# vacp2p/zerokit

Measured on AMD Instinct MI355X. Metric: RLN Groth16 proofs/sec (BN254, h=20), higher is better.
Workload: dtype u32 limbs (256-bit Montgomery integers, BN254 Fr/Fq; 8x32 and 9x29 forms)

## Files before the change

### zerokit_amd/csrc/prover.hip

```cpp
#include "prover.h"

#include <fcntl.h>
#include <stdlib.h>
#include <string.h>
#include <sys/stat.h>
#include <time.h>
#include <unistd.h>

#include <algorithm>
#include <atomic>
#include <chrono>
#include <deque>
#include <mutex>
#include <thread>

#include "prover_kernels.h"
#include "prover_plan.h"
#include "fq29.h"
#include "glv.h"
#include "pairing.h"
#include "poseidon.h"
#include "witness_ops.h"
#include "witness_lanes.h"
#include "witness_sched.h"
#include "fin29.h"

namespace rlnamd {

const char* const kProverStageNames[PROVER_STAGES] = {"witness", "matvec", "ntt",      "recode",
                                                      "msm_g1",  "msm_g2", "finalize", "values"};

struct Slot {
  DevBuf<uint32_t> err, coords, values;
  DevBuf<uint8_t> comp;
  DevBuf<Fr> V, abc;
  DevBuf<uint4> V29;
  DevBuf<int16_t> digits, digits2;
  DevBuf<G1XYZZ> part1, grp1, sums1, prod, tbl;
  DevBuf<G2XYZZ> part2, grp2, sums2;
  DevBuf<G1Affine> affA, affB1;
  DevBuf<G2Affine> affB2;
  DevBuf<uint32_t> pp_out;
  uint32_t* h_pp = nullptr;
  int mode = 0;
  DevBuf<uint32_t> inputs, rs, pp_in;
  uint8_t* h_in = nullptr;
  uint32_t* h_cone = nullptr;
  uint32_t* h_hints = nullptr;
  bool hinted = false;
  hipEvent_t evU = nullptr;
  hipEvent_t evE = nullptr;
  uint64_t ticket = 0;
  uint8_t* h_comp = nullptr;
  uint32_t* h_values = nullptr;
  uint32_t* h_err = nullptr;
  hipEvent_t evA = nullptr, evB = nullptr, evB2 = nullptr, evR = nullptr, evC = nullptr, evW = nullptr, evV = nullptr;
  hipEvent_t evX = nullptr;
  hipEvent_t evP = nullptr;
  DevBuf<uint4> pp_pow;
  hipEvent_t t[15] = {};
  bool used = false;
  bool marked = false;
  bool wiped = false;
  hipEvent_t evZ = nullptr;
  hipEvent_t free_event() const { return wiped ? evZ : evC; }
  size_t n = 0;
  uint32_t dB = 0, PB = 0, nch1 = 0, nch2 = 0;
};

static std::atomic<int> g_provers_on_device[64];

struct DeviceNeighbours {
  int fd = -1;
  void open_for(int dev) {
    char bus[64] = {0};
    if (hipDeviceGetPCIBusId(bus, sizeof bus, dev) != hipSuccess) {
      (void)hipGetLastError();
      return;
    }
    for (char* c = bus; *c; c++)
      if (*c == ':' || *c == '.') *c = '_';
    const std::string path = std::string("/dev/shm/rlnamd_") + bus + ".lock";
    fd = ::open(path.c_str(), O_RDWR | O_CREAT | O_CLOEXEC, 0666);
    if (fd < 0) return;
    (void)fchmod(fd, 0666);
    struct flock fl {};
    fl.l_type = F_RDLCK;
    fl.l_whence = SEEK_SET;
    fl.l_start = 0;
    fl.l_len = 1;
    if (fcntl(fd, F_SETLK, &fl) != 0) {
      ::close(fd);
      fd = -1;
    }
  }
  bool other_process() const {
    if (fd < 0) return false;
    struct flock fl {};
    fl.l_type = F_WRLCK;
    fl.l_whence = SEEK_SET;
    fl.l_start = 0;
    fl.l_len = 1;
    return fcntl(fd, F_GETLK, &fl) == 0 && fl.l_type != F_UNLCK;
  }
};
static std::mutex g_neigh_mu;
static DeviceNeighbours g_neigh[64];
static int g_neigh_users[64];

struct DeviceCount {
  int dev = -1;
  mutable std::chrono::steady_clock::time_point probed{};
  mutable bool other = false;
  DeviceCount() = default;
  DeviceCount(const DeviceCount&) = delete;
  DeviceCount& operator=(const DeviceCount&) = delete;
  void take() {
    int d = 0;
    if (hipGetDevice(&d) == hipSuccess && d >= 0 && d < 64) {
      dev = d;
      g_provers_on_device[d]++;
      std::lock_guard<std::mutex> lk(g_neigh_mu);
      if (g_neigh_users[d]++ == 0) g_neigh[d].open_for(d);
    }
  }
  bool other_process() const {
    if (dev < 0) return false;
    const auto now = std::chrono::steady_clock::now();
    if (now - probed > std::chrono::milliseconds(50)) {
      probed = now;
      std::lock_guard<std::mutex> lk(g_neigh_mu);
      other = g_neigh[dev].other_process();
    }
    return other;
  }
  bool shared() const { return dev >= 0 && (g_provers_on_device[dev] > 1 || other_process()); }
  ~DeviceCount() {
    if (dev < 0) return;
    g_provers_on_device[dev]--;
    std::lock_guard<std::mutex> lk(g_neigh_mu);
    if (--g_neigh_users[dev] == 0 && g_neigh[dev].fd >= 0) {
      ::close(g_neigh[dev].fd);
      g_neigh[dev].fd = -1;
    }
  }
};

struct Prover::Impl {
  hipStream_t sA = nullptr, sAb = nullptr, sA2 = nullptr, sB = nullptr, sB2 = nullptr, sC = nullptr;
  hipStream_t sV = nullptr;
  hipStream_t sW = nullptr;
  uint32_t seq = 0;
  float ms[PROVER_STAGES] = {0};
  DevBuf<unsigned long long> walk_clk;
  ProverTuning tune;
  DeviceCount device;
  DevBuf<GNode29> nodes29;
  DevBuf<uint32_t> consts29, slot2node;
  WitLanes witlanes;
  uint32_t nstore29 = 0, nprog29 = 0;

  uint32_t N = 0, NS = 0, NI = 0, nc = 0, ni = 0, n = 0;
  int logn = 0;
  DevBuf<uint32_t> sig2node;
  DevBuf<uint32_t> a_ptr, a_col, b_ptr, b_col;
  DevBuf<uint32_t> mv_long;
  uint32_t n_mv_long = 0;
  DevBuf<Fr> a_coef, b_coef;
  DevBuf<Fr> tw_f, tw_i, coset;
  DevBuf<G1Affine29> t1_29;
  DevBuf<G2Affine29> t2_29;
  DevBuf<uint32_t> sid1, sid2;
  struct Plan {
    DevBuf<uint32_t> rows, rsid, early_ids, late_ids, prows, prsid, pout;
    DevBuf<ChunkDesc> chunks, groups, segs, segchunks, segblocks, pchunks;
    uint32_t nchunks = 0, ngroups = 0, nseg = 0, n_early = 0, n_late = 0, npchunks = 0, nblocks = 0, maxblk = 0;
    void upload(const WalkPlan& W, hipStream_t s) {
      nchunks = (uint32_t)W.chunks.size();
      ngroups = (uint32_t)W.groups.size();
      nseg = W.nseg;
      n_early = (uint32_t)W.early_ids.size();
      n_late = (uint32_t)W.late_ids.size();
      npchunks = (uint32_t)W.pchunks.size();
      nblocks = W.nblocks;
      maxblk = W.maxblk;
      rows.assign(W.rows, s);
      rsid.assign(W.rsid, s);
      chunks.assign(W.chunks, s);
      groups.assign(W.groups, s);
      segs.assign(W.segs, s);
      segchunks.assign(W.segchunks, s);
      segblocks.assign(W.segblocks, s);
      early_ids.assign(W.early_ids, s);
      late_ids.assign(W.late_ids, s);
      if (npchunks) {
        prows.assign(W.prows, s);
        prsid.assign(W.prsid, s);
        pout.assign(W.pout, s);
        pchunks.assign(W.pchunks, s);
      }
      RLN_HIP(hipStreamSynchronize(s));
    }
  };
  Plan plan1[4][3], plan2[4][3];
  uint32_t max_chunks1t = 0, max_chunks2t = 0, max_blocks1t = 0, max_blocks2t = 0;
  uint32_t max_chunks1s = 0, max_chunks2s = 0, small_stride = 64;
  uint32_t max_chunks1 = 0, max_chunks2 = 0, max_groups1 = 0, max_groups2 = 0;
  uint32_t npts1 = 0, npts2 = 0, npaired1 = 0;
  std::vector<uint8_t> known;
  WitSegs segs;
  DevBuf<uint32_t> cut_node, cut_hint;
  uint32_t n_cut = 0, n_hints = 0;
  uint64_t hinted_batches = 0, hint_fallbacks = 0;
  bool no_hints_now = false;
  HintChains hints;
  WitLanes cone;
  uint32_t cone_nodes = 0;
  DevBuf<uint32_t> cone_rows;
  uint32_t cone_nk = 0, cone_cap = 0;
  uint32_t cone_stride = 0;
  DevBuf<uint4> cone_cache;
  DevBuf<uint32_t> iota96;
  std::vector<uint32_t> cone_gen, cone_free;
  std::vector<uint8_t> cone_live;
  hipEvent_t evConeSaved = nullptr;
  hipEvent_t evConeRead = nullptr, evConeRead2 = nullptr;
  uint64_t cone_batches = 0;
  uint32_t cone_tag = 0;
  uint64_t cone_handle(uint32_t e) const {
    return ((uint64_t)cone_tag << 44) | ((uint64_t)(cone_gen[e] & 0xFFFFFu) << 24) | (uint64_t)(e + 1);
  }
  uint32_t cone_entry(uint64_t h) const {
    const uint32_t idx = (uint32_t)(h & 0xFFFFFFu), gen = (uint32_t)((h >> 24) & 0xFFFFFu), tag = (uint32_t)(h >> 44);
    if (tag != cone_tag || idx == 0 || idx > cone_cap || !cone_live[idx - 1] || (cone_gen[idx - 1] & 0xFFFFFu) != gen) return 0xFFFFFFFFu;
    return idx - 1;
  }
  DevBuf<uint32_t> pp_in;
  DevBuf<uint32_t> wgiven;
  size_t wgiven_n = 0;
  InputSlots slots{};
  bool have_values_kernel = false;
  DevBuf<uint32_t> inputs, rs;
  static constexpr int NSLOT = 6;
  Slot slot[NSLOT];
  int nslot = 5;
  WinSched ws{}, ws2{};
  static constexpr uint32_t nh = GLV_HALVES;
  int cur = 0;
  Slot* last = nullptr;
  uint64_t tickets = 0;

  size_t batch_cap = 0;
  void wipe_slot(Slot& S, bool resident) {
    const size_t n = S.n ? S.n : batch_cap;
    const size_t B = batch_cap;
    if (!n) return;
    RLN_HIP(hipStreamWaitEvent(sW, S.evC, 0));
    WipeRanges WR{};
    auto flush = [&]() {
      if (!WR.count) return;
      hipLaunchKernelGGL(k_wipe_ranges, dim3(WR.first[WR.count]), dim3(64), 0, sW, WR);
      WR.count = 0;
    };
    auto zero = [&](void* dst, size_t bytes) {
      if (!bytes) return;
      if (WR.count == 16) flush();
      if (WR.count == 0) WR.first[0] = 0;
      WR.p[WR.count] = (uint4*)dst;
      WR.n16[WR.count] = (uint32_t)(bytes / 16);
      WR.first[WR.count + 1] = WR.first[WR.count] + (uint32_t)div_up(bytes / 16, 256);
      WR.count++;
    };
    if (resident) {
      zero(inputs.p, std::min(inputs.bytes(), n * (size_t)NI * 32));
      zero(rs.p, std::min(rs.bytes(), n * 64));
      if (wgiven.p) zero(wgiven.p, wgiven.bytes());
      wgiven_n = 0;
    } else {
      memset(S.h_in, 0, n * (size_t)NI * 32);
      memset(S.h_in + B * (size_t)NI * 32, 0, n * 64);
      __asm__ __volatile__("" : : "r"(S.h_in) : "memory");
      zero(S.inputs.p, n * (size_t)NI * 32);
      zero(S.rs.p, n * 64);
    }
    const uint32_t pg = div_up(n, 64);
    hipLaunchKernelGGL(k_wipe_cols, dim3(pg, nstore29), dim3(64), 0, sW, S.V.p, slot2node.p, nstore29, (uint32_t)B, (uint32_t)n);
    hipLaunchKernelGGL(k_wipe_v29, dim3(div_up(3 * n, 64), nstore29 + 1), dim3(64), 0, sW, S.V29.p, nstore29 + 1, (uint32_t)B,
                       (uint32_t)n);
    hipLaunchKernelGGL(k_wipe_cols, dim3(pg, NS), dim3(64), 0, sW, S.V.p, sig2node.p, NS, (uint32_t)B, (uint32_t)n);
    auto rows16 = [&](void* base, size_t nrows, size_t stride16, size_t n16) {
      if (!base || !nrows || !n16) return;
      hipLaunchKernelGGL(k_wipe_rows16, dim3(div_up(n16, 64), nrows), dim3(64), 0, sW, (uint4*)base, (uint32_t)nrows,
                         (uint32_t)stride16, (uint32_t)std::min(n16, stride16));
    };
    const size_t dB = S.dB ? S.dB : B;
    const size_t np = std::min<size_t>(B, (n + 63) / 64 * 64);
    for (DevBuf<int16_t>* d : {&S.digits, &S.digits2}) {
      if (!d->p) continue;
      const size_t drows = d->n / B;
      if (dB == B) rows16(d->p, drows, B / 8, np / 8);
      else zero(d->p, std::min(d->bytes(), (drows * dB * 2 + 31) / 32 * 32));
    }
    rows16(S.abc.p, S.abc.n / B, B * 2, np * 2);
    const size_t PB = S.PB ? S.PB : B;
    rows16(S.part1.p, S.PB ? S.nch1 : S.part1.n / PB, PB * (sizeof(G1XYZZ) / 16), std::min(np, PB) * (sizeof(G1XYZZ) / 16));
    rows16(S.part2.p, S.PB ? S.nch2 : S.part2.n / PB, PB * (sizeof(G2XYZZ) / 16), std::min(np, PB) * (sizeof(G2XYZZ) / 16));
    auto whole = [&](auto& buf) { if (buf.p) zero(buf.p, buf.bytes() / 32 * 32); };
    whole(S.grp1); whole(S.grp2); whole(S.sums1); whole(S.sums2); whole(S.prod); whole(S.tbl);
    whole(S.affA); whole(S.affB1); whole(S.affB2);
    flush();
    RLN_HIP(hipGetLastError());
    RLN_HIP(hipEventRecord(S.evZ, sW));
    S.wiped = true;
  }

  void sync_all() {
    RLN_HIP(hipStreamSynchronize(sA));
    RLN_HIP(hipStreamSynchronize(sAb));
    RLN_HIP(hipStreamSynchronize(sV));
    RLN_HIP(hipStreamSynchronize(sA2));
    RLN_HIP(hipStreamSynchronize(sB));
    if (sB2) RLN_HIP(hipStreamSynchronize(sB2));
    RLN_HIP(hipStreamSynchronize(sC));
    RLN_HIP(hipStreamSynchronize(sW));
  }
};

static void wait_yielding(hipEvent_t ev) {
  for (;;) {
    const hipError_t e = hipEventQuery(ev);
    if (e == hipSuccess) return;
    (void)hipGetLastError();
    if (e != hipErrorNotReady) RLN_HIP(e);
    struct timespec ts = {0, 50000};
    nanosleep(&ts, nullptr);
  }
}

static int env_int(const char* name, int dflt) {
  const char* v = getenv(name);
  return (v && *v) ? atoi(v) : dflt;
}

ProverTuning ProverTuning::from_env() {
  ProverTuning t;
  t.window_bits = env_int("RLNAMD_WINDOW_BITS", t.window_bits);
  t.slots = env_int("RLNAMD_SLOTS", t.slots);
  t.lanechunk_max = (uint32_t)std::max(0, env_int("RLNAMD_LANECHUNK", (int)t.lanechunk_max));
  t.lanechunk_walk_max = (uint32_t)std::max(0, env_int("RLNAMD_LANECHUNK_WALK", (int)t.lanechunk_walk_max));
  t.witlanes_max = (uint32_t)std::max(0, env_int("RLNAMD_WITLANES_MAX", (int)t.witlanes_max));
  t.lone = env_int("RLNAMD_LONE", -1);
  t.lone_small_max = (uint32_t)std::max(0, env_int("RLNAMD_LONE_SMALL", (int)t.lone_small_max));
  t.tiny_max = (uint32_t)std::max(0, env_int("RLNAMD_TINY", (int)t.tiny_max));
  t.ntt_lg_max = (uint32_t)std::max(0, env_int("RLNAMD_NTT_LG_MAX", (int)t.ntt_lg_max));
  t.partial_cache = (uint32_t)std::max(0, env_int("RLNAMD_PARTIAL_CACHE", (int)t.partial_cache));
  t.hint_max = (uint32_t)std::min<int>(std::max(0, env_int("RLNAMD_HINTS", (int)t.hint_max)), (int)HINT_PROOFS);
  t.hint_fault = env_int("RLNAMD_HINT_FAULT", 0);
  t.verify_lanes = env_int("RLNAMD_VERIFY_LANES", 0);
  if (t.verify_lanes != 1 && t.verify_lanes != 8) t.verify_lanes = 0;
  {
    const unsigned hw = std::thread::hardware_concurrency();
    const int dflt = hw ? (int)std::min<unsigned>(t.hint_threads, std::max(1u, hw / 2)) : (int)t.hint_threads;
    t.hint_threads = (uint32_t)std::min(std::max(1, env_int("RLNAMD_HINT_THREADS", dflt)), 64);
  }
  t.hint_max_warm = (uint32_t)std::min<int>(std::max(0, env_int("RLNAMD_HINTS_WARM", (int)t.hint_max_warm)), (int)HINT_PROOFS);
  t.hint_chains = (uint32_t)std::min(std::max(0, env_int("RLNAMD_HINT_CHAINS", (int)t.hint_chains)), 1024);
  return t;
}
std::string ProverTuning::describe() const {
  char b[768];
  snprintf(b, sizeof b,
           "window_bits=%d slots=%d lanechunk=%u lanechunk_walk=%u witlanes_max=%u tiny=%u ntt_lg_max=%u partial_cache=%u lone=%d "
           "lone_small=%u hints=%u hints_warm=%u hint_threads=%u hint_chains=%u verify_lanes=%d",
           window_bits, slots, lanechunk_max, lanechunk_walk_max, witlanes_max, tiny_max, ntt_lg_max, partial_cache, lone,
           lone_small_max, hint_max, hint_max_warm, hint_threads, hint_chains, verify_lanes);
  return b;
}
const ProverTuning& Prover::tuning() const { return d_->tune; }
int Prover::device_shared() const { return (d_->device.dev >= 0 && g_provers_on_device[d_->device.dev] > 1 ? 1 : 0) | (d_->device.other_process() ? 2 : 0); }

static uint32_t bitrev(uint32_t x, int bits) {
  uint32_t r = 0;
  for (int i = 0; i < bits; i++) r |= ((x >> i) & 1u) << (bits - 1 - i);
  return r;
}

static thread_local float g_init_ms[4];
static float ms_since(std::chrono::steady_clock::time_point t0) {
  return std::chrono::duration<float, std::milli>(std::chrono::steady_clock::now() - t0).count();
}
template <class F, class Entry>
static void build_table29(const std::vector<Affine<F>>& pts, const WinSched& ws, DevBuf<Entry>& table, hipStream_t s,
                          uint32_t npaired = 0) {
  size_t npts = pts.size();
  const size_t stride = ws.stride;
  auto t_alloc = std::chrono::steady_clock::now();
  table.alloc(npts * stride);
  g_init_ms[1] += ms_since(t_alloc);
  auto t_build = std::chrono::steady_clock::now();
  DevBuf<Affine<F>> d_pts(npts);
  d_pts.upload(pts.data(), npts, s);
  size_t per_pt = stride / 2 * sizeof(F);
  size_t slab = std::max<size_t>(2, (((size_t)4 << 30) / per_pt) & ~(size_t)1);
  slab = std::min(slab, (npts + 1) & ~(size_t)1);
  DevBuf<F> scratch(slab * stride / 2);
  DevBuf<Affine<F>> tmp(slab * stride);
  for (size_t k0 = 0; k0 < npts; k0 += slab) {
    size_t cnt = std::min(slab, npts - k0);
    const size_t nrows = cnt * ws.W;
    hipLaunchKernelGGL(k_table_build<F>, dim3((unsigned)nrows), dim3(64), 0, s, d_pts.p + k0, (uint32_t)cnt, ws, tmp.p,
                       scratch.p);
    hipLaunchKernelGGL((k_table_to29<Affine<F>, Entry>), dim3(div_up(cnt * stride, 256)), dim3(256), 0, s, tmp.p,
                       table.p + k0 * stride, cnt * stride, (uint32_t)stride, (uint32_t)k0, npaired);
    RLN_HIP(hipGetLastError());
  }
  RLN_HIP(hipStreamSynchronize(s));
  g_init_ms[2] += ms_since(t_build);
}

Prover::Prover(const uint8_t* zkey, size_t zkey_len, const uint8_t* graph, size_t graph_len, ProverConfig cfg)
    : d_(new Impl) {
  require_gpu();
  d_->device.take();
  const auto t_ctor = std::chrono::steady_clock::now();
  for (float& v : g_init_ms) v = 0;
  zk_ = parse_arkzkey(zkey, zkey_len);
  graph_ = parse_graph(graph, graph_len);
  (void)prepared(zk_);
  g_init_ms[0] = ms_since(t_ctor);
  Impl& D = *d_;
  D.tune = ProverTuning::from_env();
  const int wb = cfg.window_bits > 0 ? cfg.window_bits : D.tune.window_bits;
  D.tune.window_bits = wb;
  const int spec1 = wb % 10000, spec2 = wb / 10000 ? wb / 10000 : spec1;
  c_ = spec1 % 100;
  const int wide = spec1 / 100;
  D.ws = make_sched(c_, wide);
  D.ws2 = make_sched(spec2 % 100, spec2 >= 100 ? spec2 / 100 : (wb / 10000 ? 0 : wide));
  W_ = D.ws.W * D.nh;
  c2_ = spec2 % 100;
  W2_ = D.ws2.W * D.nh;
  B_ = ((cfg.max_batch ? cfg.max_batch : 1) + 63) / 64 * 64;
  D.batch_cap = B_;

  D.N = (uint32_t)graph_.nodes.size();
  D.NS = (uint32_t)graph_.signals.size();
  D.NI = graph_.inputs_size;
  D.nc = (uint32_t)zk_.num_constraints;
  D.ni = (uint32_t)zk_.num_instance_variables;
  if (zk_.a_query.size() != D.NS || zk_.b_g1_query.size() != D.NS || zk_.b_g2_query.size() != D.NS)
    throw Error("zkey/graph mismatch: query length != number of witness signals");
  if (zk_.gamma_abc_g1.size() != D.ni || zk_.l_query.size() + D.ni != D.NS)
    throw Error("MalformedVerifyingKey: instance/aux split does not match the witness length");
  uint32_t dom = 1;
  D.logn = 0;
  while (dom < D.nc + D.ni) {
    dom <<= 1;
    D.logn++;
  }
  D.n = dom;
  if (D.logn < 1 || D.logn > 27) throw Error("PolynomialDegreeTooLarge");
  if (zk_.h_query.size() < D.n) throw Error("zkey h_query shorter than the evaluation domain");

  {
    int lo = 0, hi = 0;
    RLN_HIP(hipDeviceGetStreamPriorityRange(&lo, &hi));
    RLN_HIP(hipStreamCreateWithPriority(&D.sW, hipStreamNonBlocking, hi));
    RLN_HIP(hipStreamCreateWithPriority(&D.sA, hipStreamNonBlocking, hi));
    RLN_HIP(hipStreamCreateWithPriority(&D.sA2, hipStreamNonBlocking, hi));
    RLN_HIP(hipStreamCreateWithPriority(&D.sAb, hipStreamNonBlocking, hi));
    RLN_HIP(hipStreamCreateWithPriority(&D.sV, hipStreamNonBlocking, hi));
    RLN_HIP(hipStreamCreateWithPriority(&D.sB, hipStreamNonBlocking, lo));
    RLN_HIP(hipStreamCreateWithPriority(&D.sC, hipStreamNonBlocking, hi));
    D.nslot = std::min(std::max(D.tune.slots, 2), (int)Impl::NSLOT);
    D.walk_clk.alloc(4);
    RLN_HIP(hipMemset(D.walk_clk.p, 0, 4 * sizeof(unsigned long long)));
    RLN_HIP(hipStreamCreateWithPriority(&D.sB2, hipStreamNonBlocking, lo));
  }
  hipStream_t s = D.sB;

  RLN_HIP(hipFuncSetAttribute((const void*)(k_sum_tree<Fq2, G2Acc29>), hipFuncAttributeMaxDynamicSharedMemorySize, SUM_TREE_LDS_G2));
  RLN_HIP(hipFuncSetAttribute((const void*)(k_sum_blocks<Fq2, G2Acc29>), hipFuncAttributeMaxDynamicSharedMemorySize, SUM_TREE_LDS_G2));
  RLN_HIP(hipFuncSetAttribute((const void*)k_witness29<false>, hipFuncAttributeMaxDynamicSharedMemorySize, WIT29_LDS_BYTES));
  D.small_stride = std::max<uint32_t>(64, (std::min<uint32_t>(D.tune.lanechunk_max, (uint32_t)B_) + 63) / 64 * 64);
  const NamedInputs named = find_named_inputs(graph_, D.ni);
  D.slots = named.slots;
  D.have_values_kernel = named.have_values_kernel;
  D.hints.configure(named, D.tune.hint_chains);
  std::vector<std::vector<uint32_t>> hint_cuts;
  std::vector<uint8_t> is_cut(D.N, 0);
  if (named.have_hint_slots && D.tune.hint_max > 0 && D.hints.count() <= 64) {
    hint_cuts = find_hint_cuts(graph_, named, D.hints);
    if (!hint_cuts.empty()) D.n_hints = D.hints.count();
    for (const auto& nodes : hint_cuts)
      for (uint32_t n : nodes) is_cut[n] = 1;
  }
  const Wit29Program W29 = compile_witness29(graph_, is_cut);
  D.nprog29 = W29.nprog;
  D.nstore29 = (uint32_t)W29.slot2node.size();
  D.nodes29.assign(W29.prog, s);
  D.slot2node.assign(W29.slot2node, s);
  D.consts29.alloc(std::max<size_t>(graph_.constants.size(), 1) * 9);
  {
    DevBuf<Fr> consts;
    if (!graph_.constants.empty()) {
      consts.assign(graph_.constants, s);
      hipLaunchKernelGGL(k_consts_to29, dim3(div_up(graph_.constants.size(), 256)), dim3(256), 0, s, consts.p,
                         D.consts29.p, (uint32_t)graph_.constants.size());
    }
    RLN_HIP(hipGetLastError());
    RLN_HIP(hipStreamSynchronize(s));
  }
  D.witlanes.build(graph_, W29.store_slot, D.nstore29, s);
  if (D.witlanes.ok && !hint_cuts.empty()) {
    const WlSegments SG = wl_segments(graph_, hint_cuts);
    D.segs.build(SG, W29.store_slot, D.nstore29, s);
    if (D.segs.ok && (D.segs.max_steps * 4 > D.witlanes.nsteps || D.segs.nseg > 256)) D.segs.ok = false;
    if (D.segs.ok) {
      D.n_cut = (uint32_t)SG.cut_nodes.size();
      D.cut_node.assign(SG.cut_nodes, s);
      D.cut_hint.assign(SG.cut_hint, s);
      RLN_HIP(hipStreamSynchronize(s));
    }
  }
  D.sig2node.assign(graph_.signals, s);

  auto csr = [&](const std::vector<SparseRow>& m, DevBuf<uint32_t>& ptr, DevBuf<uint32_t>& col, DevBuf<Fr>& coef) {
    std::vector<uint32_t> hp(D.nc + 1, 0), hc;
    std::vector<Fr> hv;
    for (uint32_t r = 0; r < D.nc; r++) {
      for (size_t k = 0; k < m[r].col.size(); k++) {
        hc.push_back(graph_.signals[m[r].col[k]]);
        hv.push_back(m[r].coeff[k]);
      }
      hp[r + 1] = (uint32_t)hc.size();
    }
    ptr.assign(hp, s);
    col.assign(hc, s);
    coef.assign(hv, s);
    RLN_HIP(hipStreamSynchronize(s));
  };
  csr(zk_.a, D.a_ptr, D.a_col, D.a_coef);
  csr(zk_.b, D.b_ptr, D.b_col, D.b_coef);
  {
    std::vector<uint32_t> lr;
    for (uint32_t r = 0; r < D.nc; r++)
      if (zk_.a[r].col.size() > MV_LONG || zk_.b[r].col.size() > MV_LONG) lr.push_back(r);
    D.n_mv_long = (uint32_t)lr.size();
    D.mv_long.assign(lr, s);
    RLN_HIP(hipStreamSynchronize(s));
  }

  {
    Fr root28 = Fr::from_canonical(FR_ROOT_2_28);
    Fr g = root28;
    for (int i = 0; i < 28 - (D.logn + 1); i++) g = g.sqr();
    Fr w = g.sqr();
    Fr wi = w.inv();
    std::vector<Fr> tf(D.n / 2), ti(D.n / 2), cs(D.n);
    Fr a = Fr::one(), b = Fr::one();
    for (uint32_t k = 0; k < D.n / 2; k++) {
      tf[k] = a;
      ti[k] = b;
      a = a * w;
      b = b * wi;
    }
    Fr ninv = Fr::from_u32(D.n).inv();
    std::vector<Fr> gp(D.n);
    Fr acc = ninv;
    for (uint32_t i = 0; i < D.n; i++) {
      gp[i] = acc;
      acc = acc * g;
    }
    for (uint32_t pos = 0; pos < D.n; pos++) cs[pos] = gp[bitrev(pos, D.logn)];
    D.tw_f.assign(tf, s);
    D.tw_i.assign(ti, s);
    D.coset.assign(cs, s);
    RLN_HIP(hipStreamSynchronize(s));
  }

  {
    std::vector<uint8_t> node_known = wl_known_nodes(graph_);
    D.known.resize(D.NS);
    for (uint32_t i = 0; i < D.NS; i++) D.known[i] = node_known[graph_.signals[i]];
    {
      std::vector<uint32_t> io(96);
      for (uint32_t i = 0; i < 96; i++) io[i] = i;
      D.iota96.assign(io, s);
      RLN_HIP(hipStreamSynchronize(s));
    }
    const long want = cfg.partial_cache >= 0 ? cfg.partial_cache : (long)D.tune.partial_cache;
    D.tune.partial_cache = (uint32_t)std::max(0l, want);
    if (D.witlanes.ok && want > 0) {
      const WlCone C = wl_cone(graph_, std::move(node_known));
      std::vector<uint32_t> rows;
      for (uint32_t i = 0; i < W29.slot2node.size(); i++)
        if (C.node_known[W29.slot2node[i]]) rows.push_back(i);
      D.cone.build(C.graph, wl_cone_store_slots(C, W29.store_slot), D.nstore29, s);
      D.cone_nodes = (uint32_t)C.node_of.size();
      if (D.cone.ok && !rows.empty()) {
        D.cone_nk = (uint32_t)rows.size();
        D.cone_rows.assign(rows, s);
        RLN_HIP(hipStreamSynchronize(s));
        D.cone_cap = (uint32_t)std::min<long>(want, (1l << 24) - 2);
        static std::atomic<uint32_t> next_tag{1};
        D.cone_tag = next_tag++ & 0xFFFFFu;
        D.cone_stride = D.cone_nk * 3 + PP_POWERS16;
        D.cone_cache.alloc((size_t)D.cone_cap * D.cone_stride);
        RLN_HIP(hipMemset(D.cone_cache.p, 0, D.cone_cache.bytes()));
        D.cone_gen.assign(D.cone_cap, 1);
        D.cone_live.assign(D.cone_cap, 0);
        for (uint32_t e = D.cone_cap; e-- > 0;) D.cone_free.push_back(e);
        RLN_HIP(hipEventCreateWithFlags(&D.evConeSaved, hipEventDisableTiming));
        RLN_HIP(hipEventCreateWithFlags(&D.evConeRead, hipEventDisableTiming));
        RLN_HIP(hipEventCreateWithFlags(&D.evConeRead2, hipEventDisableTiming));
      } else {
        D.cone.ok = false;
      }
    }
  }

  auto plan = [&](Impl::Plan& P, const std::vector<VRow>& rows, uint32_t nseg, uint32_t chunk_pts, int mode, uint32_t* max_chunks,
                  uint32_t npaired = 0, bool pair_chunks = false, uint32_t block_pts = SUM_TREE_LANES) {
    P.upload(make_walk_plan(rows, nseg, chunk_pts, mode, D.known, npaired, pair_chunks, block_pts), s);
    *max_chunks = std::max(*max_chunks, P.nchunks);
  };
  const int modes[3] = {PROVE_FULL, PROVE_PARTIAL, PROVE_FINISH};
  {
    const G1Rows R = g1_walk_rows(zk_, D.NS, D.n, D.ni);
    D.npaired1 = R.npaired;
    D.npts1 = (uint32_t)R.pts.size();
    D.sid1.assign(R.sids, s);
    for (int m : modes) {
      plan(D.plan1[PLAN_BIG][m], R.rows, 3, 16u, m, &D.max_chunks1, R.npaired, true);
      D.max_groups1 = std::max(D.max_groups1, D.plan1[PLAN_BIG][m].ngroups);
    }
    for (int m : modes) plan(D.plan1[PLAN_SMALL][m], R.rows, 3, 4u, m, &D.max_chunks1s, R.npaired);
    plan(D.plan1[PLAN_TINY][PROVE_PARTIAL], R.rows, 3, 1u, PROVE_PARTIAL, &D.max_chunks1t, R.npaired, false, SUM_TREE_LANES / 2);
    for (int m : {(int)PROVE_FULL, (int)PROVE_FINISH}) {
      plan(D.plan1[PLAN_FUSED][m], R.fused, 3, 4u, m, &D.max_chunks1s, R.npaired);
      plan(D.plan1[PLAN_TINY][m], R.fused, 3, 1u, m, &D.max_chunks1t, R.npaired, false, SUM_TREE_LANES / 2);
    }
    for (int m : modes) D.max_blocks1t = std::max(D.max_blocks1t, D.plan1[PLAN_TINY][m].nblocks);
    build_table29<Fq, G1Affine29>(R.pts, D.ws, D.t1_29, s, R.npaired);
  }
  {
    const G2Rows R = g2_walk_rows(zk_, D.NS, D.n);
    D.npts2 = (uint32_t)R.pts.size();
    D.sid2.assign(R.dsid, s);
    for (int m : modes) {
      plan(D.plan2[PLAN_BIG][m], R.rows, 1, 8u, m, &D.max_chunks2);
      D.max_groups2 = std::max(D.max_groups2, D.plan2[PLAN_BIG][m].ngroups);
    }
    for (int m : modes) plan(D.plan2[PLAN_SMALL][m], R.rows, 1, 2u, m, &D.max_chunks2s);
    for (int m : modes) {
      plan(D.plan2[PLAN_TINY][m], R.rows, 1, 1u, m, &D.max_chunks2t, 0, false, SUM_TREE_LANES / 2);
      D.max_blocks2t = std::max(D.max_blocks2t, D.plan2[PLAN_TINY][m].nblocks);
    }
    build_table29<Fq2, G2Affine29>(R.pts, D.ws2, D.t2_29, s);
  }

  poseidon_dev();

  const size_t B = B_;
  D.inputs.alloc(B * D.NI * 8);
  D.rs.alloc(B * 16);
  D.pp_in.alloc(B * 80);
  RLN_HIP(hipMemsetAsync(D.pp_in.p, 0, D.pp_in.bytes(), s));
  RLN_HIP(hipMemsetAsync(D.inputs.p, 0, D.inputs.bytes(), s));
  RLN_HIP(hipMemsetAsync(D.rs.p, 0, D.rs.bytes(), s));
  for (int si = 0; si < D.nslot; si++) {
    Slot& S = D.slot[si];
    S.err.alloc(B);
    S.coords.alloc(B * 64);
    S.values.alloc(B * 40);
    S.comp.alloc(B * 128);
    S.V.alloc((size_t)D.N * B);
    S.V29.alloc(((size_t)D.nstore29 + 1) * 3 * B);
    S.abc.alloc(3 * (size_t)D.n * B);
    S.digits.alloc((size_t)(3 * D.NS + D.n + 4) * D.nh * D.ws.W * B);
    S.digits2.alloc((size_t)(D.NS + 3) * D.nh * D.ws2.W * B);
    S.part1.alloc(std::max({(size_t)D.max_chunks1 * B, (size_t)D.max_chunks1s * D.small_stride,
                            (size_t)D.max_chunks1t * TINY_STRIDE}));
    S.grp1.alloc(std::max((size_t)D.max_groups1 * B, (size_t)D.max_blocks1t * TINY_STRIDE));
    S.sums1.alloc(3 * D.nh * B);
    S.part2.alloc(std::max({(size_t)D.max_chunks2 * B, (size_t)D.max_chunks2s * D.small_stride,
                            (size_t)D.max_chunks2t * TINY_STRIDE}));
    S.grp2.alloc(std::max((size_t)D.max_groups2 * B, (size_t)D.max_blocks2t * TINY_STRIDE));
    S.sums2.alloc(D.nh * B);
    S.prod.alloc(2 * B);
    S.tbl.alloc(2 * 16 * B);
    S.affA.alloc(B);
    S.affB1.alloc(B);
    S.affB2.alloc(B);
    S.pp_out.alloc(B * 80);
    S.inputs.alloc(B * D.NI * 8);
    S.rs.alloc(B * 16);
    S.pp_in.alloc(B * 80);
    RLN_HIP(hipMemsetAsync(S.inputs.p, 0, S.inputs.bytes(), s));
    RLN_HIP(hipMemsetAsync(S.rs.p, 0, S.rs.bytes(), s));
    RLN_HIP(hipMemsetAsync(S.pp_in.p, 0, S.pp_in.bytes(), s));
    RLN_HIP(hipHostMalloc((void**)&S.h_in, B * ((size_t)D.NI * 32 + 64 + 320), hipHostMallocDefault));
    RLN_HIP(hipHostMalloc((void**)&S.h_cone, B * 4, hipHostMallocDefault));
    RLN_HIP(hipHostMalloc((void**)&S.h_hints, (size_t)HINT_PROOFS * 64 * 32, hipHostMallocDefault));
    RLN_HIP(hipEventCreateWithFlags(&S.evU, hipEventDisableTiming));
    RLN_HIP(hipEventCreateWithFlags(&S.evE, hipEventDisableTiming));
    RLN_HIP(hipHostMalloc((void**)&S.h_pp, B * 320, hipHostMallocDefault));
    RLN_HIP(hipHostMalloc((void**)&S.h_comp, B * 128, hipHostMallocDefault));
    RLN_HIP(hipHostMalloc((void**)&S.h_values, B * 160, hipHostMallocDefault));
    RLN_HIP(hipHostMalloc((void**)&S.h_err, B * 4, hipHostMallocDefault));
    RLN_HIP(hipEventCreateWithFlags(&S.evA, hipEventDisableTiming));
    RLN_HIP(hipEventCreateWithFlags(&S.evB, hipEventDisableTiming));
    RLN_HIP(hipEventCreateWithFlags(&S.evB2, hipEventDisableTiming));
    RLN_HIP(hipEventCreateWithFlags(&S.evR, hipEventDisableTiming));
    RLN_HIP(hipEventCreateWithFlags(&S.evW, hipEventDisableTiming));
    RLN_HIP(hipEventCreateWithFlags(&S.evX, hipEventDisableTiming));
    RLN_HIP(hipEventCreateWithFlags(&S.evP, hipEventDisableTiming));
    S.pp_pow.alloc((size_t)std::min<size_t>(B, 96) * PP_POWERS16);
    RLN_HIP(hipEventCreateWithFlags(&S.evV, hipEventDisableTiming));
    RLN_HIP(hipEventCreateWithFlags(&S.evC, hipEventDisableTiming));
    RLN_HIP(hipEventCreateWithFlags(&S.evZ, hipEventDisableTiming));
    for (auto& e : S.t) RLN_HIP(hipEventCreate(&e));
    RLN_HIP(hipMemsetAsync(S.digits.p, 0, S.digits.bytes(), s));
    RLN_HIP(hipMemsetAsync(S.digits2.p, 0, S.digits2.bytes(), s));
  }
  RLN_HIP(hipStreamSynchronize(s));
  g_init_ms[3] = ms_since(t_ctor) - g_init_ms[0] - g_init_ms[1] - g_init_ms[2];
  for (int k = 0; k < 4; k++) init_ms_[k] = g_init_ms[k];
}

Prover::~Prover() {
  if (!d_) return;
  Impl& D = *d_;
  for (hipStream_t st : {D.sA, D.sAb, D.sA2, D.sB, D.sB2, D.sC, D.sV, D.sW})
    if (st) (void)hipStreamSynchronize(st);
  try {
    if (D.sW) {
      for (int k = 0; k < D.nslot; k++)
        if (D.slot[k].used && !D.slot[k].wiped && D.slot[k].evC) D.wipe_slot(D.slot[k], D.slot[k].ticket == 0);
      if (D.cone_cache.p)
        hipLaunchKernelGGL(k_wipe_bytes, dim3(div_up(D.cone_cache.bytes() / 16, 256)), dim3(64), 0, D.sW, D.cone_cache.p,
                           (uint32_t)(D.cone_cache.bytes() / 16));
      (void)hipStreamSynchronize(D.sW);
    }
  } catch (...) {
  }
  for (Slot& S : D.slot) {
    if (S.h_pp) (void)hipHostFree(S.h_pp);
    if (S.h_in) (void)hipHostFree(S.h_in);
    if (S.h_cone) (void)hipHostFree(S.h_cone);
    if (S.h_hints) (void)hipHostFree(S.h_hints);
    if (S.evU) (void)hipEventDestroy(S.evU);
    if (S.evE) (void)hipEventDestroy(S.evE);
    if (S.h_comp) (void)hipHostFree(S.h_comp);
    if (S.h_values) (void)hipHostFree(S.h_values);
    if (S.h_err) (void)hipHostFree(S.h_err);
    for (hipEvent_t e : {S.evA, S.evB, S.evB2, S.evR, S.evC, S.evW, S.evV, S.evX, S.evZ, S.evP})
      if (e) (void)hipEventDestroy(e);
    for (auto& e : S.t)
      if (e) (void)hipEventDestroy(e);
  }
  for (hipEvent_t e : {D.evConeSaved, D.evConeRead, D.evConeRead2})
    if (e) (void)hipEventDestroy(e);
  for (hipStream_t st : {D.sA, D.sAb, D.sA2, D.sB, D.sB2, D.sC, D.sV, D.sW})
    if (st) (void)hipStreamDestroy(st);
}

size_t Prover::table_bytes() const { return d_->t1_29.bytes() + d_->t2_29.bytes(); }
size_t Prover::g1_rows() const { return d_->npts1; }
size_t Prover::g2_rows() const { return d_->npts2; }

void Prover::upload(size_t n, const uint8_t* inputs, const uint8_t* rs) {
  if (n > B_) throw Error("batch larger than the prover workspace (max_batch)");
  Impl& D = *d_;
  D.sync_all();
  RLN_HIP(hipMemcpyAsync(D.inputs.p, inputs, n * D.NI * 32, hipMemcpyHostToDevice, D.sA));
  RLN_HIP(hipMemcpyAsync(D.rs.p, rs, n * 64, hipMemcpyHostToDevice, D.sA));
  RLN_HIP(hipStreamSynchronize(D.sA));
}

void Prover::upload_witness(size_t n, const uint8_t* w_le) {
  if (n > B_) throw Error("batch larger than the prover workspace (max_batch)");
  Impl& D = *d_;
  D.sync_all();
  size_t words = n * (size_t)D.NS * 8;
  if (D.wgiven.n < words) D.wgiven.alloc(words);
  RLN_HIP(hipMemcpyAsync(D.wgiven.p, w_le, words * 4, hipMemcpyHostToDevice, D.sA));
  RLN_HIP(hipStreamSynchronize(D.sA));
  D.wgiven_n = n;
}

template <bool DIF>
static void launch_ntt(Fr* data, const Fr* tw, int logn, const Fr* final_scale, uint32_t B, uint32_t nb, hipStream_t s) {
  int s0 = 0;
  while (s0 < logn) {
    const int rem = logn - s0;
    const int K = rem > 3 ? 3 : rem;
    const uint32_t groups = (1u << logn) >> K;
    dim3 block(64, 1), grid(div_up(nb, 64), groups, 3);
    const Fr* sc = (s0 + K == logn) ? final_scale : nullptr;
    switch (K) {
      case 1: hipLaunchKernelGGL((k_ntt_pass<1, DIF>), grid, block, 0, s, data, tw, logn, s0, sc, B, nb); break;
      case 2: hipLaunchKernelGGL((k_ntt_pass<2, DIF>), grid, block, 0, s, data, tw, logn, s0, sc, B, nb); break;
      default: hipLaunchKernelGGL((k_ntt_pass<3, DIF>), grid, block, 0, s, data, tw, logn, s0, sc, B, nb); break;
    }
    RLN_HIP(hipGetLastError());
    s0 += K;
  }
}

void Prover::run_async(size_t n, int mode) { enqueue(n, mode, nullptr, nullptr, nullptr); }

uint64_t Prover::submit(size_t n, const uint8_t* inputs, const uint8_t* rs, int mode, const uint8_t* partial320) {
  if (n == 0) throw Error("empty batch");
  if (!inputs || !rs) throw Error("submit: inputs and rs are required");
  if (mode == PROVE_FINISH && !partial320) throw Error("submit: finish mode needs the partial points");
  return enqueue(n, mode, inputs, rs, partial320);
}

uint64_t Prover::submit_finish(size_t n, const uint8_t* inputs, const uint8_t* rs, const uint8_t* partial320,
                               const uint64_t* handles) {
  if (n == 0) throw Error("empty batch");
  if (!inputs || !rs || !partial320) throw Error("submit_finish: inputs, rs and the partial points are required");
  return enqueue(n, PROVE_FINISH, inputs, rs, partial320, handles);
}

uint32_t Prover::hint_words() const {
  const Impl& D = *d_;
  return D.segs.ok && D.tune.hint_max > 0 ? D.n_hints * 8 : 0;
}

void Prover::hints_for(const uint8_t* inputs, uint32_t* hints) const {
  const Impl& D = *d_;
  if (!D.segs.ok) throw Error("hints_for: this prover interprets no segments (hint_words() is 0)");
  Fr hv[64];
  D.hints.hints(inputs, hv);
  for (uint32_t j = 0; j < D.n_hints; j++) hv[j].to_canonical(hints + (size_t)j * 8);
}

uint64_t Prover::submit_hinted(size_t n, const uint8_t* inputs, const uint8_t* rs, const uint32_t* hints) {
  if (n == 0) throw Error("empty batch");
  if (!inputs || !rs) throw Error("submit: inputs and rs are required");
  return enqueue(n, PROVE_FULL, inputs, rs, nullptr, nullptr, hint_words() && n <= HINT_PROOFS ? hints : nullptr);
}

void Prover::collect_partial_cached(uint64_t ticket, size_t n, uint8_t* partial320, uint64_t* handles, uint32_t* errors) {
  Impl& D = *d_;
  ticket = settle_hints(ticket);
  Slot* Sp = nullptr;
  for (int k = 0; k < D.nslot; k++)
    if (D.slot[k].used && D.slot[k].ticket == ticket && ticket != 0) Sp = &D.slot[k];
  if (!Sp) throw Error("collect: unknown or expired ticket (its workspace slot has been reused)");
  Slot& S = *Sp;
  if (S.mode != PROVE_PARTIAL) throw Error("collect_partial_cached: not a partial-proof batch");
  if (n > S.n) throw Error("collect: more proofs requested than the batch holds");
  if (S.wiped) throw Error("collect_partial_cached: the batch has been wiped");
  RLN_HIP(hipEventSynchronize(S.evC));
  size_t cached = 0;
  for (size_t i = 0; i < n; i++) {
    if (handles) handles[i] = 0;
    if (!handles || !D.cone.ok || D.cone_free.empty() || S.h_err[i] != 0 || cached != i) continue;
    const uint32_t e = D.cone_free.back();
    D.cone_free.pop_back();
    D.cone_live[e] = 1;
    S.h_cone[i] = e;
    handles[i] = D.cone_handle(e);
    cached++;
  }
  if (cached) {
    RLN_HIP(hipStreamWaitEvent(D.sW, S.evC, 0));
    hipLaunchKernelGGL(k_cone_save, dim3(div_up(D.cone_nk * 3, 256), (uint32_t)cached), dim3(256), 0, D.sW, S.V29.p, D.cone_rows.p,
                       D.cone_nk, (uint32_t)B_, S.h_cone, D.cone_cache.p, D.cone_stride);
    launch_pp_powers(D.sW, S.pp_out.p, S.h_cone, D.cone_cache.p, D.cone_stride, D.cone_nk * 3, (uint32_t)cached);
    RLN_HIP(hipGetLastError());
    RLN_HIP(hipEventRecord(D.evConeSaved, D.sW));
  }
  collect(ticket, n, nullptr, nullptr, errors, nullptr, partial320, true);
}

void Prover::release_partial(const uint64_t* handles, size_t n) {
  Impl& D = *d_;
  if (!D.cone_cap || !handles) return;
  bool any = false;
  for (size_t i = 0; i < n; i++) {
    const uint32_t e = D.cone_entry(handles[i]);
    if (e == 0xFFFFFFFFu) continue;
    if (!any) {
      RLN_HIP(hipStreamWaitEvent(D.sW, D.evConeRead, 0));
      RLN_HIP(hipStreamWaitEvent(D.sW, D.evConeRead2, 0));
    }
    any = true;
    uint4* at = D.cone_cache.p + (size_t)e * D.cone_stride;
    hipLaunchKernelGGL(k_wipe_bytes, dim3(div_up(D.cone_stride, 256)), dim3(64), 0, D.sW, at, D.cone_stride);
    D.cone_live[e] = 0;
    D.cone_gen[e]++;
    D.cone_free.push_back(e);
  }
  if (any) {
    RLN_HIP(hipGetLastError());
    RLN_HIP(hipEventRecord(D.evConeSaved, D.sW));
  }
}

void Prover::hint_stats(uint64_t out[HINT_STATS_FIELDS]) const {
  const Impl& D = *d_;
  out[0] = D.segs.ok ? D.segs.nseg : 0;
  out[1] = D.segs.ok ? D.n_hints : 0;
  out[2] = D.segs.ok ? D.segs.max_steps : 0;
  out[3] = D.witlanes.ok ? D.witlanes.nsteps : 0;
  out[4] = D.hinted_batches;
  out[5] = D.hint_fallbacks;
  out[6] = D.hints.hits();
}

void Prover::partial_cache_info(uint64_t out[PARTIAL_CACHE_FIELDS]) {
  Impl& D = *d_;
  for (int k = 0; k < PARTIAL_CACHE_FIELDS; k++) out[k] = 0;
  out[0] = D.cone_cap;
  out[1] = D.cone_cap - D.cone_free.size();
  out[2] = (uint64_t)D.cone_stride * 16;
  out[4] = D.cone_batches;
  out[5] = D.cone_nodes;
  out[6] = D.cone.ok ? D.cone.nsteps : 0;
  out[7] = D.witlanes.ok ? D.witlanes.nsteps : 0;
  if (!D.cone_cap) return;
  sync();
  RLN_HIP(hipStreamSynchronize(D.sW));
  DevBuf<unsigned long long> cnt(1);
  RLN_HIP(hipMemsetAsync(cnt.p, 0, cnt.bytes(), D.sC));
  for (uint32_t e = 0; e < D.cone_cap; e++)
    if (!D.cone_live[e])
      hipLaunchKernelGGL(k_count_nonzero16, dim3(64), dim3(256), 0, D.sC, (const uint4*)(D.cone_cache.p + (size_t)e * D.cone_stride),
                         (size_t)D.cone_stride, cnt.p);
  RLN_HIP(hipGetLastError());
  unsigned long long h = 0;
  RLN_HIP(hipMemcpyAsync(&h, cnt.p, sizeof h, hipMemcpyDeviceToHost, D.sC));
  RLN_HIP(hipStreamSynchronize(D.sC));
  out[3] = h;
}

uint64_t Prover::settle_hints(uint64_t ticket) {
  Impl& D = *d_;
  Slot* Sp = nullptr;
  for (int k = 0; k < D.nslot; k++)
    if (D.slot[k].used && D.slot[k].ticket == ticket && ticket != 0) Sp = &D.slot[k];
  if (!Sp || !Sp->hinted) return ticket;
  Slot& S = *Sp;
  RLN_HIP(hipEventSynchronize(S.evC));
  S.hinted = false;
  bool bad = false;
  for (size_t i = 0; i < S.n; i++) bad = bad || (S.h_err[i] & WERR_HINT) != 0;
  if (!bad) return ticket;
  D.hint_fallbacks++;
  D.no_hints_now = true;
  uint64_t again = 0;
  try {
    const uint8_t* in = S.h_in;
    again = enqueue(S.n, S.mode, in, in + B_ * (size_t)D.NI * 32, S.mode == PROVE_FINISH ? in + B_ * ((size_t)D.NI * 32 + 64) : nullptr, nullptr);
  } catch (...) {
    D.no_hints_now = false;
    throw;
  }
  D.no_hints_now = false;
  if (!S.wiped) D.wipe_slot(S, false);
  return again;
}

void Prover::collect(uint64_t ticket, size_t n, uint8_t* proofs, uint8_t* values, uint32_t* errors, uint8_t* coords,
                     uint8_t* partial320, bool wipe_after) {
  Impl& D = *d_;
  ticket = settle_hints(ticket);
  Slot* Sp = nullptr;
  for (int k = 0; k < D.nslot; k++)
    if (D.slot[k].used && D.slot[k].ticket == ticket && ticket != 0) Sp = &D.slot[k];
  if (!Sp) throw Error("collect: unknown or expired ticket (its workspace slot has been reused)");
  Slot& S = *Sp;
  if (n > S.n) throw Error("collect: more proofs requested than the batch holds");
  if (S.n > D.tune.lanechunk_max) wait_yielding(S.evC); else RLN_HIP(hipEventSynchronize(S.evC));
  if (S.mode == PROVE_PARTIAL) {
    if (partial320) memcpy(partial320, S.h_pp, n * 320);
  } else {
    if (proofs) memcpy(proofs, S.h_comp, n * 128);
    if (values) {
      if (D.have_values_kernel)
        memcpy(values, S.h_values, n * 160);
      else if (D.ni == 6) {
        std::vector<uint8_t> pub;
        fetch_public_slot(&S, n, &pub);
        memcpy(values, pub.data(), n * 160);
      } else
        memset(values, 0, n * 160);
    }
    if (coords) RLN_HIP(hipMemcpy(coords, S.coords.p, n * 256, hipMemcpyDeviceToHost));
  }
  if (errors) memcpy(errors, S.h_err, n * 4);
  if (wipe_after && !S.wiped) D.wipe_slot(S, false);
}

void Prover::wipe(uint64_t ticket) {
  Impl& D = *d_;
  if (ticket == 0) {
    D.sync_all();
    if (D.last) D.wipe_slot(*D.last, true);
    RLN_HIP(hipStreamSynchronize(D.sW));
    return;
  }
  for (int k = 0; k < D.nslot; k++)
    if (D.slot[k].used && D.slot[k].ticket == ticket) {
      RLN_HIP(hipEventSynchronize(D.slot[k].evC));
      if (!D.slot[k].wiped) D.wipe_slot(D.slot[k], false);
      return;
    }
}

void Prover::collect_public(uint64_t ticket, size_t n, std::vector<uint8_t>* out_le) {
  Impl& D = *d_;
  if (ticket != settle_hints(ticket)) throw Error("collect_public: the batch was run again (collect it first)");
  for (int k = 0; k < D.nslot; k++)
    if (D.slot[k].used && D.slot[k].ticket == ticket && ticket != 0) {
      if (n > D.slot[k].n) throw Error("collect: more proofs requested than the batch holds");
      if (D.slot[k].wiped) throw Error("collect_public: the batch has been wiped (collect it with wipe_after = false first)");
      RLN_HIP(hipEventSynchronize(D.slot[k].evC));
      fetch_public_slot(&D.slot[k], n, out_le);
      return;
    }
  throw Error("collect: unknown or expired ticket (its workspace slot has been reused)");
}

int Prover::slots() const { return d_->nslot; }

void Prover::prove_stream(size_t n, const uint8_t* inputs, const uint8_t* rs, uint8_t* proofs, uint8_t* values,
                          uint32_t* errors) {
  size_t at = 0;
  prove_stream_from([&](size_t* off, size_t* cnt) {
    if (at >= n) return false;
    *off = at;
    *cnt = std::min(B_, n - at);
    at += *cnt;
    return true;
  }, inputs, rs, proofs, values, errors);
}

void Prover::prove_stream_from(const ChunkSource& next, const uint8_t* inputs, const uint8_t* rs, uint8_t* proofs,
                               uint8_t* values, uint32_t* errors, int max_in_flight) {
  Impl& D = *d_;
  struct Pending { uint64_t ticket; size_t off, cnt; };
  std::deque<Pending> q;
  const size_t NIB = (size_t)D.NI * 32;
  const int depth = max_in_flight > 0 ? std::min(max_in_flight, D.nslot) : D.nslot;
  auto take = [&]() {
    Pending f = q.front();
    q.pop_front();
    collect(f.ticket, f.cnt, proofs ? proofs + f.off * 128 : nullptr, values ? values + f.off * 160 : nullptr,
            errors ? errors + f.off : nullptr);
  };
  try {
    size_t off = 0, cnt = 0;
    for (;;) {
      if ((int)q.size() == depth) take();
      if (!next(&off, &cnt)) break;
      if (cnt == 0) continue;
      if (cnt > B_) throw Error("prove_stream: a chunk larger than the prover workspace (max_batch)");
      q.push_back({submit(cnt, inputs + off * NIB, rs + off * 64), off, cnt});
    }
    while (!q.empty()) take();
  } catch (...) {
    D.sync_all();
    for (int k = 0; k < D.nslot; k++)
      if (D.slot[k].used && !D.slot[k].wiped) D.wipe_slot(D.slot[k], false);
    D.sync_all();
    throw;
  }
}

template <class F>
static void on_hint_threads(size_t n, size_t nth, F&& per_proof) {
  std::vector<std::thread> helpers;
  std::atomic<bool> failed{false};
  auto strand = [&](size_t k) {
    try {
      for (size_t i = k; i < n; i += nth) per_proof(i);
    } catch (...) {
      failed = true;
    }
  };
  try {
    for (size_t k = 1; k < nth; k++) helpers.emplace_back(strand, k);
  } catch (...) {
    const size_t started = helpers.size() + 1;
    for (size_t k = started; k < nth; k++) strand(k);
  }
  strand(0);
  for (std::thread& th : helpers) th.join();
  if (failed) throw Error("out of memory while hashing the hints of a batch");
}

uint64_t Prover::enqueue(size_t n, int mode, const uint8_t* h_inputs, const uint8_t* h_rs, const uint8_t* h_pp320,
                         const uint64_t* cone_handles, const uint32_t* pre_hints) {
  if (n == 0) return 0;
  if (n > B_) throw Error("batch larger than the prover workspace (max_batch)");
  if (mode < PROVE_FULL || mode > PROVE_FINISH) throw Error("unknown prover mode");
  Impl& D = *d_;
  const ProverTuning& T = D.tune;
  BatchQuery q;
  q.n = n;
  q.mode = mode;
  q.inputs = h_inputs != nullptr;
  q.partial_points = h_pp320 != nullptr;
  q.handles = cone_handles != nullptr;
  q.pre_hints = pre_hints != nullptr;
  q.idle = T.lone >= 0 || n <= T.lone_small_max || !D.last || hipEventQuery(D.last->evC) == hipSuccess;
  (void)hipGetLastError();
  q.shared = D.device.shared();
  q.no_hints_now = D.no_hints_now;
  q.witlanes_ok = D.witlanes.ok;
  q.segs_ok = D.segs.ok;
  q.cone_ok = D.cone.ok;
  q.have_values_kernel = D.have_values_kernel;
  q.ni = D.ni;
  q.logn = D.logn;
  q.capacity = B_;
  q.small_stride = D.small_stride;
  BatchShape sh = batch_shape(q, T);
  std::vector<uint32_t> cone_entries;
  for (size_t i = 0; i < n && sh.cone; i++) {
    const uint32_t e = D.cone_entry(cone_handles[i]);
    if (e != 0xFFFFFFFFu) {
      cone_entries.push_back(e);
    } else {
      q.handles = false;
      sh = batch_shape(q, T);
    }
  }
  std::vector<HintChains::Probe> probes;
  const size_t hint_nth = std::min<size_t>(std::max<size_t>(n, 1), std::max<uint32_t>(1u, T.hint_threads));
  if (sh.probe_chains) {
    probes.resize(n);
    for (size_t i = 0; i < 2 && sh.hinted; i++) {
      D.hints.probe(h_inputs + i * (size_t)D.NI * 32, &probes[i]);
      sh.hinted = probes[i].found;
    }
  }
  if (sh.probe_chains && sh.hinted) {
    on_hint_threads(n, hint_nth, [&](size_t i) {
      if (i >= 2) D.hints.probe(h_inputs + i * (size_t)D.NI * 32, &probes[i]);
    });
    size_t to_hash = 0;
    for (const HintChains::Probe& pr : probes) to_hash += pr.found ? 0 : 1;
    sh.hinted = 2 * to_hash <= 5 * hint_nth;
  }
  if (!sh.hinted) probes.clear();
  const bool lone = sh.lone, small = sh.small, wl_used = sh.wl_used, cone = sh.cone, hinted = sh.hinted, early = sh.early,
             fused = sh.fused, tiny = sh.tiny, tiny_partial = sh.tiny_partial, walk_lp = sh.walk_lp;
  const Impl::Plan &P1 = D.plan1[sh.plan1][mode], &P2 = D.plan2[sh.plan2][mode];
  const uint32_t PB = sh.PB, dB = sh.dB;
  Slot& S = D.slot[D.cur];
  S.dB = dB;
  S.PB = PB;
  S.nch1 = P1.nchunks;
  S.nch2 = P2.nchunks;
  const bool streamed = h_inputs != nullptr;
  if (streamed) {
    if (D.wgiven_n) throw Error("upload_witness applies to the resident-input run that follows it, not to submit");
    if (S.used) RLN_HIP(hipEventSynchronize(S.free_event()));
    memcpy(S.h_in, h_inputs, n * (size_t)D.NI * 32);
    memcpy(S.h_in + B_ * (size_t)D.NI * 32, h_rs, n * 64);
    if (h_pp320) memcpy(S.h_in + B_ * ((size_t)D.NI * 32 + 64), h_pp320, n * 320);
  }
  const uint32_t* in_p = streamed ? S.inputs.p : D.inputs.p;
  const uint32_t* rs_p = streamed ? S.rs.p : D.rs.p;
  const uint32_t* pp_p = (streamed && h_pp320) ? S.pp_in.p : D.pp_in.p;
  S.mode = mode;
  S.ticket = streamed ? ++D.tickets : 0;
  D.cur = (D.cur + 1) % D.nslot;
  const uint32_t sq = D.seq++;
  const bool idle = !D.last || hipEventQuery(D.last->evC) == hipSuccess;
  (void)hipGetLastError();
  hipStream_t sA = (!idle && (sq & 1)) ? D.sAb : D.sA;
  const uint32_t B = (uint32_t)B_, nb = (uint32_t)n;
  hipStream_t sA2 = !early ? D.sA2 : sh.g2_on_front ? D.sB2 : sA;
  const uint32_t pg = div_up(nb, 64);
  const uint32_t nbp = pg * 64;
  auto d2h = [&](void* host, const void* dev, size_t bytes, hipStream_t st) {
    if (!small && bytes % 16 == 0)
      hipLaunchKernelGGL(k_stage_in, dim3(div_up(bytes / 16, 64)), dim3(64), 0, st, (const uint4*)dev, (uint4*)host, (uint32_t)(bytes / 16));
    else
      RLN_HIP(hipMemcpyAsync(host, dev, bytes, hipMemcpyDeviceToHost, st));
  };
  auto walk1 = [&](hipStream_t st, const uint32_t* ids, uint32_t cnt) {
    if (!cnt) return;
    const uint32_t blocks = div_up(cnt, 8) * 8 * pg;
    if (!small) {
      const PairPlan pp{P1.prows.p, P1.prsid.p, P1.pchunks.p, P1.pout.p, P1.npchunks};
      const uint32_t pblocks = div_up(P1.npchunks, 8) * 8 * (2 * pg);
      hipLaunchKernelGGL((k_msm29<G1Acc29, G1Affine29, G1XYZZ, 4>), dim3(blocks + pblocks), dim3(64), 0, st, D.t1_29.p,
                         P1.rsid.p, P1.rows.p, P1.chunks.p, cnt, S.digits.p, S.part1.p, D.ws, dB, pg, D.nh, D.walk_clk.p, ids,
                         0u, pp);
    } else if (walk_lp) {
      hipLaunchKernelGGL((k_msm29<G1Acc29, G1Affine29, G1XYZZ, 4>), dim3(blocks), dim3(64), 0, st, D.t1_29.p, P1.rsid.p,
                         P1.rows.p, P1.chunks.p, cnt, S.digits.p, S.part1.p, D.ws, dB, pg, D.nh, nullptr, ids, PB);
    } else {
      hipLaunchKernelGGL((k_msm29<G1Acc29, G1Affine29, G1XYZZ, 2, true>), dim3(div_up(cnt, 64), nb), dim3(64), 0, st,
                         D.t1_29.p, P1.rsid.p, P1.rows.p, P1.chunks.p, cnt, S.digits.p, S.part1.p, D.ws, dB, PB, D.nh,
                         nullptr, ids);
    }
  };
  if (S.used) RLN_HIP(hipStreamWaitEvent(sA, S.free_event(), 0));
  if (streamed) {
    auto h2d = [&](void* dst, const uint8_t* src, size_t bytes) {
      hipLaunchKernelGGL(k_stage_in, dim3(div_up(bytes / 16, 64)), dim3(64), 0, sA, (const uint4*)src, (uint4*)dst,
                         (uint32_t)(bytes / 16));
    };
    h2d(S.inputs.p, S.h_in, n * (size_t)D.NI * 32);
    h2d(S.rs.p, S.h_in + B_ * (size_t)D.NI * 32, n * 64);
    if (h_pp320) h2d(S.pp_in.p, S.h_in + B_ * ((size_t)D.NI * 32 + 64), n * 320);
    RLN_HIP(hipGetLastError());
    RLN_HIP(hipEventRecord(S.evU, sA));
  }
  const bool marks = !small;
  S.marked = marks;
#define MARK(i, stream)                                   \
  do {                                                    \
    if (marks) RLN_HIP(hipEventRecord(S.t[i], stream));   \
  } while (0)
  if (cone) memcpy(S.h_cone, cone_entries.data(), n * sizeof(uint32_t));
  S.hinted = hinted;
  if (hinted) {
    if (pre_hints)
      memcpy(S.h_hints, pre_hints, n * (size_t)D.n_hints * 32);
    else
      on_hint_threads(n, hint_nth, [&](size_t i) {
        Fr hv[64];
        D.hints.hints(h_inputs + i * (size_t)D.NI * 32, hv, probes.empty() ? nullptr : &probes[i]);
        for (uint32_t j = 0; j < D.n_hints; j++) hv[j].to_canonical(S.h_hints + (i * D.n_hints + j) * 8);
      });
    if (T.hint_fault > 0 && (uint32_t)T.hint_fault <= D.n_hints) S.h_hints[(size_t)(T.hint_fault - 1) * 8] ^= 1u;
    D.hinted_batches++;
  }
  if (fused && mode == PROVE_FINISH) {
    if (S.used) RLN_HIP(hipStreamWaitEvent(D.sC, S.free_event(), 0));
    RLN_HIP(hipStreamWaitEvent(D.sC, S.evU, 0));
    if (cone) {
      RLN_HIP(hipStreamWaitEvent(D.sC, D.evConeSaved, 0));
      launch_pp_smul(D.sC, D.cone_cache.p, S.h_cone, D.cone_stride, D.cone_nk * 3, rs_p, S.prod.p, nb);
      RLN_HIP(hipEventRecord(D.evConeRead2, D.sC));
    } else {
      launch_pp_powers(D.sC, pp_p, D.iota96.p, S.pp_pow.p, PP_POWERS16, 0, nb);
      launch_pp_smul(D.sC, S.pp_pow.p, D.iota96.p, PP_POWERS16, 0, rs_p, S.prod.p, nb);
    }
    RLN_HIP(hipGetLastError());
    RLN_HIP(hipEventRecord(S.evP, D.sC));
  }
  MARK(1, sA);
  if (cone) {
    RLN_HIP(hipStreamWaitEvent(sA, D.evConeSaved, 0));
    hipLaunchKernelGGL(k_cone_restore, dim3(div_up(D.cone_nk * 3, 256), nb), dim3(256), 0, sA, D.cone_cache.p, D.cone_rows.p,
                       D.cone_nk, B, S.h_cone, S.V29.p, D.cone_stride);
    RLN_HIP(hipEventRecord(D.evConeRead, sA));
    D.cone.launch(sA, in_p, D.NI, S.V29.p, S.err.p, B, nb);
    D.cone_batches++;
  } else if (hinted) {
    hipLaunchKernelGGL(k_wipe_bytes, dim3(1), dim3(64), 0, sA, (uint4*)S.err.p, (uint32_t)div_up(nb * 4, 16));
    D.segs.launch(sA, in_p, D.NI, S.h_hints, S.V29.p, S.err.p, B, nb);
  } else if (wl_used) {
    D.witlanes.launch(sA, in_p, D.NI, S.V29.p, S.err.p, B, nb);
  } else {
    hipLaunchKernelGGL(k_witness29<false>, dim3(pg), dim3(64), WIT29_LDS_BYTES, sA, D.nodes29.p, D.nprog29,
                       D.consts29.p, (uint32_t)graph_.constants.size(), in_p, D.NI, S.V29.p, S.err.p, B, nbp, nullptr);
  }
  if (small)
    hipLaunchKernelGGL(k_v29_to_fr, dim3(div_up(D.nstore29, 64), nb), dim3(64, 1), 0, sA, S.V29.p, D.slot2node.p,
                       D.nstore29, S.V.p, B, nb, 1u);
  else
    hipLaunchKernelGGL(k_v29_to_fr, dim3(pg, D.nstore29), dim3(64, 1), 0, sA, S.V29.p, D.slot2node.p, D.nstore29, S.V.p,
                       B, nbp);
  if (hinted)
    hipLaunchKernelGGL(k_hint_check, dim3(div_up(D.n_cut, 64), nb), dim3(64), 0, sA, S.V.p, D.cut_node.p, D.cut_hint.p, D.n_cut,
                       S.h_hints, D.n_hints, B, S.err.p);
  if (D.wgiven_n) {
    if (D.wgiven_n != n || mode != PROVE_FULL) throw Error("upload_witness: the next run must be a full proof of the same batch");
    hipLaunchKernelGGL(k_scatter_witness, dim3(pg, div_up(D.NS, 4)), dim3(64, 4), 0, sA, D.wgiven.p, D.sig2node.p,
                       D.NS, S.V.p, S.err.p, B, nb);
    D.wgiven_n = 0;
  }
  RLN_HIP(hipEventRecord(S.evX, sA));
  if (early) {
    hipStream_t sR1 = sA, sR3 = lone ? D.sB : sA;
    hipLaunchKernelGGL(k_recode, dim3(div_up(D.NS + 3, 64), nb), dim3(64, 1), 0, sR1, S.V.p, D.sig2node.p, D.NS,
                       S.abc.p, D.n, rs_p, D.ws, D.ws2, S.digits.p, S.digits2.p, B, nb, 1u, 1u, dB);
    if (lone) {
      RLN_HIP(hipEventRecord(S.evW, sA));
      RLN_HIP(hipStreamWaitEvent(D.sB, S.evW, 0));
    }
    if (fused)
      hipLaunchKernelGGL(k_recode, dim3(div_up(2 * D.NS + 1, 64), nb), dim3(64, 1), 0, sR3, S.V.p, D.sig2node.p, D.NS,
                         S.abc.p, D.n, rs_p, D.ws, D.ws2, S.digits.p, S.digits2.p, B, nb, 3u, 1u, dB);
    if (!lone) {
      RLN_HIP(hipEventRecord(S.evW, sA));
      RLN_HIP(hipStreamWaitEvent(D.sB, S.evW, 0));
      RLN_HIP(hipStreamWaitEvent(D.sB2, S.evW, 0));
    }
    MARK(14, D.sB);
    walk1(D.sB, P1.early_ids.p, P1.n_early);
    RLN_HIP(hipEventRecord(S.evE, D.sB));
  }
  MARK(2, sA);
  if (sA2 != sA) RLN_HIP(hipStreamWaitEvent(sA2, S.evX, 0));
  MARK(12, sA2);
  if (mode != PROVE_PARTIAL) {
    CsrView A{D.a_ptr.p, D.a_col.p, D.a_coef.p}, Bm{D.b_ptr.p, D.b_col.p, D.b_coef.p};
    if (small)
      hipLaunchKernelGGL(k_matvec<true>, dim3(div_up(D.n, 64) + D.n_mv_long, nb), dim3(64, 1), 0, sA2, A, Bm, S.V.p,
                         D.sig2node.p, D.nc, D.ni, D.n, S.abc.p, B, nb, D.mv_long.p, div_up(D.n, 64));
    else
      hipLaunchKernelGGL(k_matvec<false>, dim3(pg, D.n), dim3(64, 1), 0, sA2, A, Bm, S.V.p, D.sig2node.p, D.nc,
                         D.ni, D.n, S.abc.p, B, nbp);
  }
  MARK(3, sA2);
  if (mode != PROVE_PARTIAL) {
    if (sh.ntt_lds) {
      const dim3 grid(nb, D.n >> 9, 3);
      if (D.logn > 9) hipLaunchKernelGGL(k_ntt_edge<true>, grid, dim3(256), 0, sA2, S.abc.p, D.tw_i.p, D.logn, B, nb);
      hipLaunchKernelGGL(k_ntt_mid, grid, dim3(256), 0, sA2, S.abc.p, D.tw_i.p, D.tw_f.p, D.logn, D.coset.p, B, nb);
      if (D.logn > 9) hipLaunchKernelGGL(k_ntt_edge<false>, grid, dim3(256), 0, sA2, S.abc.p, D.tw_f.p, D.logn, B, nb);
      RLN_HIP(hipGetLastError());
    } else {
      launch_ntt<true>(S.abc.p, D.tw_i.p, D.logn, D.coset.p, B, nbp, sA2);
      launch_ntt<false>(S.abc.p, D.tw_f.p, D.logn, nullptr, B, nbp, sA2);
    }
    if (!early)
      hipLaunchKernelGGL(k_hquot, dim3(pg, D.n), dim3(64, 1), 0, sA2, S.abc.p, D.n, B, nbp, 0u);
  }
  MARK(4, sA2);
  hipStream_t sR = sA2;
  MARK(5, sR);
  if (early)
    hipLaunchKernelGGL(k_recode, dim3(div_up(D.n, 64), nb), dim3(64, 1), 0, sR, S.V.p, D.sig2node.p, D.NS, S.abc.p, D.n,
                       rs_p, D.ws, D.ws2, S.digits.p, S.digits2.p, B, nb, 2u, 2u, dB);
  else
    hipLaunchKernelGGL(k_recode, dim3(pg, D.NS + D.n + 3), dim3(64, 1), 0, sR, S.V.p, D.sig2node.p, D.NS,
                       S.abc.p, D.n, rs_p, D.ws, D.ws2, S.digits.p, S.digits2.p, B, nbp, 0u, 0u, dB);
  MARK(6, sR);
  if (!early) {
    RLN_HIP(hipEventRecord(S.evA, sA2));
    RLN_HIP(hipStreamWaitEvent(D.sB, S.evA, 0));
    MARK(14, D.sB);
  }
  hipStream_t s2 = sh.g2_on_front ? sA : D.sB2;
  if (!early) {
    RLN_HIP(hipEventRecord(S.evR, D.sB));
    RLN_HIP(hipStreamWaitEvent(D.sB2, S.evR, 0));
  }
  if (early) {
    walk1(sA2, P1.late_ids.p, P1.n_late);
    RLN_HIP(hipEventRecord(S.evR, sA2));
    RLN_HIP(hipStreamWaitEvent(D.sB, S.evR, 0));
  } else {
    walk1(D.sB, nullptr, P1.nchunks);
  }
  MARK(7, D.sB);
  MARK(11, s2);
  if (P2.nchunks) {
    uint32_t blocks = div_up(P2.nchunks, 8) * 8 * pg;
    if (walk_lp)
      hipLaunchKernelGGL((k_msm29<G2Acc29, G2Affine29, G2XYZZ, 2>), dim3(blocks), dim3(64), 0, s2, D.t2_29.p, P2.rsid.p,
                         P2.rows.p, P2.chunks.p, P2.nchunks, S.digits2.p, S.part2.p, D.ws2, dB, pg, D.nh, nullptr, nullptr, PB);
    else if (tiny)
      hipLaunchKernelGGL((k_msm29<G2AccPair29, G2Affine29, G2XYZZ, 1, true>), dim3(div_up(2 * P2.nchunks, 64), nb), dim3(64), 0, s2,
                         D.t2_29.p, P2.rsid.p, P2.rows.p, P2.chunks.p, P2.nchunks, S.digits2.p, S.part2.p, D.ws2, dB, PB, D.nh,
                         nullptr);
    else if (small)
      hipLaunchKernelGGL((k_msm29<G2Acc29, G2Affine29, G2XYZZ, 1, true>), dim3(div_up(P2.nchunks, 64), nb), dim3(64), 0, s2,
                         D.t2_29.p, P2.rsid.p, P2.rows.p, P2.chunks.p, P2.nchunks, S.digits2.p, S.part2.p, D.ws2, dB, PB, D.nh,
                         nullptr);
    else
      hipLaunchKernelGGL((k_msm29<G2Acc29, G2Affine29, G2XYZZ, 2>), dim3(blocks), dim3(64), 0, s2, D.t2_29.p, P2.rsid.p,
                         P2.rows.p, P2.chunks.p, P2.nchunks, S.digits2.p, S.part2.p, D.ws2, dB, pg, D.nh,
                         D.walk_clk.p ? D.walk_clk.p + 2 : nullptr);
  }
  MARK(8, s2);
  RLN_HIP(hipEventRecord(S.evB, D.sB));
  RLN_HIP(hipEventRecord(S.evB2, s2));
  hipStream_t sV = D.sV;
  if (S.used) {
    RLN_HIP(hipStreamWaitEvent(D.sC, S.free_event(), 0));
    RLN_HIP(hipStreamWaitEvent(sV, S.free_event(), 0));
  }
  if (streamed) RLN_HIP(hipStreamWaitEvent(sV, S.evU, 0));
  MARK(0, sV);
  if (sh.values_w) {
    RLN_HIP(hipStreamWaitEvent(sV, S.evX, 0));
    hipLaunchKernelGGL(k_values_from_witness, dim3(pg, 5), dim3(64), 0, sV, S.V.p, D.sig2node.p, B, nbp, S.values.p);
  } else if (D.have_values_kernel)
    hipLaunchKernelGGL(k_proof_values, dim3(pg), dim3(64), 0, sV, in_p, D.NI, D.slots, poseidon_view(2),
                       poseidon_view(3), poseidon_view(4), S.values.p, nbp);
  MARK(13, sV);
  const bool fin_pp = mode == PROVE_FINISH;
  const TaskSel all4 = task_sel({0, 1, 2, 3}), all3 = task_sel({0, 1, 2});
  hipStream_t sF = D.sC;
  auto sum1 = [&](hipStream_t st, std::initializer_list<uint32_t> segs) {
    const TaskSel sel = task_sel(segs);
    const uint32_t ns = (uint32_t)segs.size();
    if (tiny) {
      hipLaunchKernelGGL((k_sum_blocks<Fq, G1AccPair29>), dim3(nb, ns, std::max(P1.maxblk, 1u)), dim3(SUM_TREE_LANES), SUM_TREE_LDS_G1 / 2, st, S.part1.p, P1.segchunks.p,
                         P1.segblocks.p, S.grp1.p, PB, sel);
      hipLaunchKernelGGL((k_sum_tree<Fq, G1AccPair29>), dim3(nb, ns), dim3(SUM_TREE_LANES), SUM_TREE_LDS_G1 / 2, st, S.grp1.p, P1.segblocks.p, S.sums1.p, B, PB, sel);
    } else {
      hipLaunchKernelGGL((k_sum_tree<Fq, G1Acc29>), dim3(nb, ns), dim3(SUM_TREE_LANES), SUM_TREE_LDS_G1, st, S.part1.p, P1.segchunks.p, S.sums1.p, B, PB, sel);
    }
  };
  auto sum2 = [&](hipStream_t st) {
    const TaskSel sel = task_sel({0, 1, 2, 3, 4, 5});
    if (tiny) {
      hipLaunchKernelGGL((k_sum_blocks<Fq2, G2AccPair29>), dim3(nb, P2.nseg, std::max(P2.maxblk, 1u)), dim3(SUM_TREE_LANES), SUM_TREE_LDS_G2 / 2, st, S.part2.p,
                         P2.segchunks.p, P2.segblocks.p, S.grp2.p, PB, sel);
      hipLaunchKernelGGL((k_sum_tree<Fq2, G2AccPair29>), dim3(nb, P2.nseg), dim3(SUM_TREE_LANES), SUM_TREE_LDS_G2 / 2, st, S.grp2.p, P2.segblocks.p, S.sums2.p, B, PB, sel);
    } else {
      hipLaunchKernelGGL((k_sum_tree<Fq2, G2Acc29>), dim3(nb, P2.nseg), dim3(SUM_TREE_LANES), SUM_TREE_LDS_G2, st, S.part2.p, P2.segchunks.p, S.sums2.p, B, PB, sel);
    }
  };
  if (early) {
    RLN_HIP(hipStreamWaitEvent(D.sA2, S.evE, 0));
    if (fused) {
      sum1(D.sA2, {0, 3});
      if (fin_pp) hipLaunchKernelGGL(k_add_partial, dim3(pg, 1), dim3(64), 0, D.sA2, S.sums1.p, S.sums2.p, pp_p, B, nbp, task_sel({0}), (const G1XYZZ*)nullptr);
    } else {
      sum1(D.sA2, {0, 1, 3, 4});
      if (fin_pp) hipLaunchKernelGGL(k_add_partial, dim3(pg, 2), dim3(64), 0, D.sA2, S.sums1.p, S.sums2.p, pp_p, B, nbp, task_sel({0, 1}), (const G1XYZZ*)nullptr);
      hipLaunchKernelGGL(k_glv_fold, dim3(pg, 2), dim3(64), 0, D.sA2, S.sums1.p, S.sums2.p, 3u, B, nbp, task_sel({0, 1}));
      hipLaunchKernelGGL(k_fin_affine, dim3(pg, 2), dim3(64), 0, D.sA2, S.sums1.p, S.sums2.p, S.affA.p, S.affB1.p,
                         S.affB2.p, B, nbp, task_sel({0, 1}));
      launch_fin_smul29(D.sA2, S.affA.p, S.affB1.p, rs_p, S.prod.p, B, nb);
    }
    RLN_HIP(hipGetLastError());
    RLN_HIP(hipEventRecord(S.evA, D.sA2));
    hipStream_t sG = lone ? s2 : D.sC;
    if (!lone) RLN_HIP(hipStreamWaitEvent(D.sC, S.evB2, 0));
    sum2(sG);
    if (fin_pp) hipLaunchKernelGGL(k_add_partial, dim3(pg, 1), dim3(64), 0, sG, S.sums1.p, S.sums2.p, pp_p, B, nbp, task_sel({3}), (const G1XYZZ*)nullptr);
    hipLaunchKernelGGL(k_fin_out_b2, dim3(pg), dim3(64), 0, sG, S.sums2.p, S.coords.p, S.comp.p, B, nbp);
    if (lone) RLN_HIP(hipEventRecord(S.evB2, s2));
    RLN_HIP(hipEventRecord(S.evV, sV));
    hipStream_t sAC = lone ? sA2 : sF;
    if (lone) {
      sF = sA;
      MARK(9, sF);
      RLN_HIP(hipStreamWaitEvent(sAC, S.evE, 0));
    } else {
      MARK(9, sF);
      RLN_HIP(hipStreamWaitEvent(sF, S.evB, 0));
    }
    sum1(sAC, {2, 5});
    if (fin_pp) hipLaunchKernelGGL(k_add_partial, dim3(pg, 1), dim3(64), 0, sAC, S.sums1.p, S.sums2.p, pp_p, B, nbp, task_sel({2}), (const G1XYZZ*)nullptr);
    if (fin_pp && fused) {
      RLN_HIP(hipStreamWaitEvent(sAC, S.evP, 0));
      hipLaunchKernelGGL(k_add_partial, dim3(pg, 1), dim3(64), 0, sAC, S.sums1.p, S.sums2.p, pp_p, B, nbp, task_sel({4}), (const G1XYZZ*)S.prod.p);
    }
    RLN_HIP(hipStreamWaitEvent(sAC, S.evA, 0));
    if (fused)
      hipLaunchKernelGGL(k_fin_out_ac_fused, dim3(pg), dim3(64), 0, sAC, S.sums1.p, S.affA.p, S.coords.p, S.comp.p, B, nbp);
    else
      hipLaunchKernelGGL(k_fin_out_ac, dim3(pg), dim3(64), 0, sAC, S.sums1.p, S.prod.p, S.affA.p, S.coords.p, S.comp.p, B, nbp);
    if (lone) {
      RLN_HIP(hipEventRecord(S.evA, sAC));
      RLN_HIP(hipStreamWaitEvent(sF, S.evA, 0));
    }
    RLN_HIP(hipStreamWaitEvent(sF, S.evV, 0));
  } else {
    if (tiny_partial) {
      sum2(s2);
      RLN_HIP(hipEventRecord(S.evB2, s2));
    }
    RLN_HIP(hipEventRecord(S.evV, sV));
    RLN_HIP(hipStreamWaitEvent(D.sC, S.evV, 0));
    RLN_HIP(hipStreamWaitEvent(D.sC, S.evB, 0));
    if (tiny_partial) sum1(D.sC, {0, 1, 2, 3, 4, 5});
    RLN_HIP(hipStreamWaitEvent(D.sC, S.evB2, 0));
    MARK(9, D.sC);
  }
  if (early || tiny_partial) {
  } else if (small) {
    sum1(D.sC, {0, 1, 2, 3, 4, 5});
    sum2(D.sC);
  } else {
    if (P1.ngroups)
      hipLaunchKernelGGL(k_sum_ranges<Fq>, dim3(pg, P1.ngroups), dim3(64), 0, D.sC, S.part1.p, P1.groups.p, P1.ngroups,
                         S.grp1.p, B, nbp);
    if (P2.ngroups)
      hipLaunchKernelGGL(k_sum_ranges<Fq2>, dim3(pg, P2.ngroups), dim3(64), 0, D.sC, S.part2.p, P2.groups.p, P2.ngroups,
                         S.grp2.p, B, nbp);
    hipLaunchKernelGGL(k_sum_ranges<Fq>, dim3(pg, P1.nseg), dim3(64), 0, D.sC, S.grp1.p, P1.segs.p, P1.nseg, S.sums1.p, B, nbp);
    hipLaunchKernelGGL(k_sum_ranges<Fq2>, dim3(pg, P2.nseg), dim3(64), 0, D.sC, S.grp2.p, P2.segs.p, P2.nseg, S.sums2.p, B, nbp);
  }
  if (!early)
    hipLaunchKernelGGL(k_glv_fold, dim3(pg, 4), dim3(64), 0, D.sC, S.sums1.p, S.sums2.p, 3u, B, nbp, all4);
  if (mode == PROVE_PARTIAL) {
    hipLaunchKernelGGL(k_partial_out, dim3(pg, 4), dim3(64), 0, D.sC, S.sums1.p, S.sums2.p, S.pp_out.p, B, nbp);
    RLN_HIP(hipGetLastError());
    d2h(S.h_pp, S.pp_out.p, n * 320, D.sC);
  } else {
    if (!early) {
      if (mode == PROVE_FINISH)
        hipLaunchKernelGGL(k_add_partial, dim3(pg, 4), dim3(64), 0, D.sC, S.sums1.p, S.sums2.p, pp_p, B, nbp, all4, (const G1XYZZ*)nullptr);
      hipLaunchKernelGGL(k_fin_affine, dim3(pg, 3), dim3(64), 0, D.sC, S.sums1.p, S.sums2.p, S.affA.p, S.affB1.p,
                         S.affB2.p, B, nbp, all3);
      hipLaunchKernelGGL(k_fin_smul, dim3(pg, 2), dim3(64), 0, D.sC, S.affA.p, S.affB1.p, rs_p, S.tbl.p, S.prod.p, B,
                         nbp);
      hipLaunchKernelGGL(k_fin_out, dim3(pg), dim3(64), 0, sF, S.sums1.p, S.prod.p, S.affA.p, S.affB2.p, S.coords.p,
                         S.comp.p, B, nbp);
    }
    RLN_HIP(hipGetLastError());
    d2h(S.h_comp, S.comp.p, n * 128, sF);
    d2h(S.h_values, S.values.p, n * 160, sF);
  }
  d2h(S.h_err, S.err.p, n * 4, sF);
  MARK(10, sF);
  RLN_HIP(hipEventRecord(S.evC, sF));
  S.used = true;
  S.wiped = false;
  S.n = n;
  D.last = &S;
  return S.ticket;
}

void Prover::sync() { sync_measure(false); }

void Prover::sync_measure(bool last_only) {
  Impl& D = *d_;
  D.sync_all();
  if (D.last) {
    const int pairs[PROVER_STAGES][2] = {{1, 2}, {12, 3}, {3, 4}, {5, 6}, {14, 7}, {11, 8}, {9, 10}, {0, 13}};
    float acc[PROVER_STAGES] = {0};
    int cnt = 0;
    for (int k = 0; k < D.nslot; k++) {
      Slot& S = D.slot[k];
      if (!S.used || !S.marked || S.mode != D.last->mode || S.n != D.last->n || (last_only && &S != D.last)) continue;
      for (int i = 0; i < PROVER_STAGES; i++) {
        float ms = 0;
        RLN_HIP(hipEventElapsedTime(&ms, S.t[pairs[i][0]], S.t[pairs[i][1]]));
        acc[i] += ms;
      }
      cnt++;
    }
    for (int i = 0; i < PROVER_STAGES; i++) D.ms[i] = cnt ? acc[i] / cnt : 0.f;
  }
}

void Prover::run(size_t n, int mode) {
  sync();
  run_async(n, mode);
  sync_measure(true);
}

void Prover::upload_partial(size_t n, const uint8_t* coords320) {
  if (n > B_) throw Error("batch larger than the prover workspace (max_batch)");
  Impl& D = *d_;
  D.sync_all();
  RLN_HIP(hipMemcpyAsync(D.pp_in.p, coords320, n * 320, hipMemcpyHostToDevice, D.sA));
  RLN_HIP(hipStreamSynchronize(D.sA));
}

void Prover::download_partial(size_t n, uint8_t* coords320) {
  Impl& D = *d_;
  sync();
  if (!D.last || D.last->mode != PROVE_PARTIAL || n > D.last->n) throw Error("the last run was not a partial-proof run");
  memcpy(coords320, D.last->h_pp, n * 320);
}

const std::vector<uint8_t>& Prover::known_mask() const { return d_->known; }

void Prover::stage_ms(float out[PROVER_STAGES]) const {
  for (int i = 0; i < PROVER_STAGES; i++) out[i] = d_->ms[i];
}

void Prover::walk_clock_mhz(double out[2]) {
  Impl& D = *d_;
  sync();
  unsigned long long h[4] = {0, 0, 0, 0};
  if (D.walk_clk.p) {
    RLN_HIP(hipMemcpy(h, D.walk_clk.p, sizeof(h), hipMemcpyDeviceToHost));
    RLN_HIP(hipMemset(D.walk_clk.p, 0, sizeof(h)));
  }
  for (int g = 0; g < 2; g++) out[g] = h[2 * g + 1] ? 100.0 * (double)h[2 * g] / (double)h[2 * g + 1] : 0.0;
}

void Prover::download(size_t n, ProofOut* out) {
  if (n > B_) throw Error("batch larger than the prover workspace (max_batch)");
  Impl& D = *d_;
  sync();
  if (!D.last) throw Error("no resident run to read from");
  Slot& S = *D.last;
  std::vector<uint32_t> coords(n * 64);
  RLN_HIP(hipMemcpyAsync(coords.data(), S.coords.p, n * 256, hipMemcpyDeviceToHost, D.sC));
  RLN_HIP(hipStreamSynchronize(D.sC));
  std::vector<uint8_t> pub;
  const bool from_public = !D.have_values_kernel && D.ni == 6;
  if (from_public) fetch_public(n, &pub);
  for (size_t i = 0; i < n; i++) {
    memcpy(out[i].compressed, S.h_comp + i * 128, 128);
    memcpy(out[i].coords, coords.data() + i * 64, 256);
    if (D.have_values_kernel)
      memcpy(out[i].values, S.h_values + i * 40, 160);
    else if (from_public)
      memcpy(out[i].values, pub.data() + i * 160, 160);
    else
      memset(out[i].values, 0, 160);
    out[i].error = S.h_err[i];
  }
}

void Prover::fetch_public(size_t n, std::vector<uint8_t>* out_le) {
  Impl& D = *d_;
  sync();
  if (!D.last || n > B_) throw Error("no resident run to read from");
  fetch_public_slot(D.last, n, out_le);
}

void Prover::fetch_public_slot(void* slot, size_t n, std::vector<uint8_t>* out_le) {
  Impl& D = *d_;
  Slot& S = *(Slot*)slot;
  const uint32_t npub = D.ni - 1;
  DevBuf<uint32_t> tmp(n * npub * 8);
  hipLaunchKernelGGL(k_public_signals, dim3(div_up(n, 64), div_up(npub, 4)), dim3(64, 4), 0, D.sC, S.V.p,
                     D.sig2node.p, npub, (uint32_t)B_, (uint32_t)n, tmp.p);
  out_le->resize(n * npub * 32);
  RLN_HIP(hipMemcpyAsync(out_le->data(), tmp.p, out_le->size(), hipMemcpyDeviceToHost, D.sC));
  RLN_HIP(hipStreamSynchronize(D.sC));
}

void Prover::fetch_witness(size_t p, std::vector<uint8_t>* w_le) {
  Impl& D = *d_;
  sync();
  if (!D.last || p >= B_) throw Error("no resident run to read from");
  DevBuf<uint32_t> tmp((size_t)D.NS * 8);
  hipLaunchKernelGGL(k_gather_col, dim3(div_up(D.NS, 256)), dim3(256), 0, D.sC, D.last->V.p, D.sig2node.p, D.NS,
                     (uint32_t)B_, (uint32_t)p, tmp.p);
  w_le->resize((size_t)D.NS * 32);
  RLN_HIP(hipMemcpyAsync(w_le->data(), tmp.p, w_le->size(), hipMemcpyDeviceToHost, D.sC));
  RLN_HIP(hipStreamSynchronize(D.sC));
}

void Prover::fetch_h(size_t p, std::vector<uint8_t>* h_le) {
  Impl& D = *d_;
  sync();
  if (!D.last || p >= B_) throw Error("no resident run to read from");
  DevBuf<uint32_t> tmp((size_t)D.n * 8);
  hipLaunchKernelGGL(k_gather_col, dim3(div_up(D.n, 256)), dim3(256), 0, D.sC, D.last->abc.p, (const uint32_t*)nullptr,
                     D.n, (uint32_t)B_, (uint32_t)p, tmp.p);
  h_le->resize((size_t)D.n * 32);
  RLN_HIP(hipMemcpyAsync(h_le->data(), tmp.p, h_le->size(), hipMemcpyDeviceToHost, D.sC));
  RLN_HIP(hipStreamSynchronize(D.sC));
}

void Prover::residue(uint64_t out[RESIDUE_FIELDS]) {
  Impl& D = *d_;
  sync();
  if (!D.last) throw Error("no run to read from");
  Slot& S = *D.last;
  DevBuf<unsigned long long> cnt(RESIDUE_FIELDS);
  RLN_HIP(hipMemsetAsync(cnt.p, 0, cnt.bytes(), D.sC));
  auto count = [&](int k, const void* p, size_t bytes) {
    if (p && bytes >= 16)
      hipLaunchKernelGGL(k_count_nonzero16, dim3(2048), dim3(256), 0, D.sC, (const uint4*)p, bytes / 16, cnt.p + k);
  };
  count(0, S.digits.p, S.digits.bytes());
  count(1, S.digits2.p, S.digits2.bytes());
  count(2, S.abc.p, S.abc.bytes());
  count(3, S.part1.p, S.part1.bytes());
  count(4, S.part2.p, S.part2.bytes());
  for (auto* b : {&S.grp1, &S.sums1, &S.prod, &S.tbl}) count(3, b->p, b->bytes());
  for (auto* b : {&S.grp2, &S.sums2}) count(4, b->p, b->bytes());
  count(3, S.affA.p, S.affA.bytes());
  count(3, S.affB1.p, S.affB1.bytes());
  count(4, S.affB2.p, S.affB2.bytes());
  count(5, S.inputs.p, S.inputs.bytes());
  count(5, S.rs.p, S.rs.bytes());
  RLN_HIP(hipGetLastError());
  unsigned long long h[RESIDUE_FIELDS];
  RLN_HIP(hipMemcpyAsync(h, cnt.p, sizeof h, hipMemcpyDeviceToHost, D.sC));
  RLN_HIP(hipStreamSynchronize(D.sC));
  for (int k = 0; k < RESIDUE_FIELDS; k++) out[k] = h[k];
}

}
```

### zerokit_amd/csrc/prover_plan.cpp

```cpp
#include "prover_plan.h"

#include <string.h>

#include <algorithm>

#include "glv.h"
#include "poseidon.h"
#include "witness_sched.h"

namespace rlnamd {

WinSched make_sched(int c, int wide) {
  if (c < 2 || c > 16 || wide < 0 || c + (wide > 0 ? 1 : 0) > 16) throw Error("window bits must be in [2, 16]");
  WinSched ws{};
  int W = (GlvParams::HALF_BITS - wide + c - 1) / c;
  if (wide > W) throw Error("more wide windows than windows");
  if (W > 32) throw Error("window bits too small: more than 32 windows");
  ws.W = W;
  uint32_t bit = 0, off = 0;
  for (int j = 0; j < W; j++) {
    int cw = c + (j < wide ? 1 : 0);
    ws.cw[j] = (uint8_t)cw;
    ws.bo[j] = (uint16_t)bit;
    ws.ro[j] = off;
    bit += cw;
    off += 1u << (cw - 1);
  }
  ws.stride = off;
  return ws;
}

NamedInputs find_named_inputs(const Graph& graph, uint32_t ni) {
  NamedInputs R;
  auto find = [&](const char* name, uint32_t want_len, uint32_t* off) {
    auto it = graph.input_mapping.find(name);
    if (it == graph.input_mapping.end() || it->second.second != want_len) return false;
    *off = it->second.first;
    return true;
  };
  InputSlots& sl = R.slots;
  sl.depth = graph.tree_depth;
  uint32_t unused = 0;
  R.hint_msgs = graph.max_out;
  R.have_hint_slots = find("identitySecret", 1, &sl.secret) && find("userMessageLimit", 1, &sl.limit) &&
                      find("messageId", graph.max_out, &R.hint_msg_off) && find("pathElements", graph.tree_depth, &sl.path) &&
                      find("identityPathIndex", graph.tree_depth, &sl.path_idx) && find("x", 1, &sl.x) &&
                      find("externalNullifier", 1, &sl.ext) &&
                      (graph.max_out == 1 || find("selectorUsed", graph.max_out, &unused));
  R.have_values_kernel = R.have_hint_slots && graph.max_out == 1 && ni == 6;
  if (R.have_values_kernel) sl.msg_id = R.hint_msg_off;
  return R;
}

static Fr read_input(const uint8_t* in_le, uint32_t slot) {
  uint32_t c[8];
  memcpy(c, in_le + 32 * (size_t)slot, 32);
  return Fr::from_canonical(c);
}

void HintChains::probe(const uint8_t* in_le, Probe* pr) const {
  const InputSlots& slots = in_.slots;
  const Fr secret = read_input(in_le, slots.secret);
  pr->idc = poseidon_hash_host(poseidon_host_params(2), &secret);
  uint64_t fp[2] = {0x9E3779B97F4A7C15ull, 0xC2B2AE3D27D4EB4Full};
  auto mix = [&](const uint32_t* w, int n) {
    for (int k = 0; k < n; k++) {
      fp[0] = (fp[0] ^ w[k]) * 0xFF51AFD7ED558CCDull;
      fp[0] ^= fp[0] >> 29;
      fp[1] = (fp[1] + w[k]) * 0xC4CEB9FE1A85EC53ull;
      fp[1] ^= fp[1] >> 31;
    }
  };
  auto mix_slots = [&](uint32_t first, uint32_t count) {
    for (uint32_t k = 0; k < count; k++) {
      uint32_t w[8];
      memcpy(w, in_le + 32 * (size_t)(first + k), 32);
      mix(w, 8);
    }
  };
  mix(pr->idc.v, 8);
  mix_slots(slots.limit, 1);
  mix_slots(slots.path, slots.depth);
  mix_slots(slots.path_idx, slots.depth);
  pr->fp[0] = fp[0];
  pr->fp[1] = fp[1];
  pr->found = false;
  if (entries_) {
    std::lock_guard<std::mutex> lk(mu_);
    for (const Entry& e : cache_)
      if (e.fp[0] == fp[0] && e.fp[1] == fp[1] && e.chain.size() == slots.depth) pr->found = true;
  }
}

void HintChains::hints(const uint8_t* in_le, Fr* out, const Probe* pr) const {
  const InputSlots& slots = in_.slots;
  const PoseidonParams &P3 = poseidon_host_params(3), &P4 = poseidon_host_params(4);
  Probe mine;
  if (!pr) {
    probe(in_le, &mine);
    pr = &mine;
  }
  const Fr secret = read_input(in_le, slots.secret), limit = read_input(in_le, slots.limit);
  const Fr idc = pr->idc;
  out[0] = idc;
  const uint64_t fp[2] = {pr->fp[0], pr->fp[1]};
  bool found = false;
  if (entries_) {
    std::lock_guard<std::mutex> lk(mu_);
    for (Entry& e : cache_)
      if (e.fp[0] == fp[0] && e.fp[1] == fp[1] && e.chain.size() == slots.depth) {
        for (uint32_t l = 0; l < slots.depth; l++) out[1 + l] = e.chain[l];
        e.stamp = ++clock_;
        hits_++;
        found = true;
        break;
      }
  }
  if (!found) {
    Fr in2[2] = {idc, limit};
    Fr node = poseidon_hash_host(P3, in2);
    out[1] = node;
    for (uint32_t l = 0; l < slots.depth; l++) {
      const Fr e = read_input(in_le, slots.path + l);
      const bool right = !read_input(in_le, slots.path_idx + l).is_zero();
      in2[0] = right ? e : node;
      in2[1] = right ? node : e;
      node = poseidon_hash_host(P3, in2);
      if (l + 1 < slots.depth) out[2 + l] = node;
    }
    if (entries_) {
      std::lock_guard<std::mutex> lk(mu_);
      Entry* slot = nullptr;
      if (cache_.size() < entries_) {
        cache_.emplace_back();
        slot = &cache_.back();
      } else {
        slot = &cache_[0];
        for (Entry& e : cache_)
          if (e.stamp < slot->stamp) slot = &e;
      }
      slot->fp[0] = fp[0];
      slot->fp[1] = fp[1];
      slot->stamp = ++clock_;
      slot->chain.assign(out + 1, out + 1 + slots.depth);
    }
  }
  for (uint32_t k = 0; k < in_.hint_msgs; k++) {
    const Fr in3[3] = {secret, read_input(in_le, slots.ext), read_input(in_le, in_.hint_msg_off + k)};
    out[slots.depth + 1 + k] = poseidon_hash_host(P4, in3);
  }
}

uint64_t HintChains::hits() const {
  std::lock_guard<std::mutex> lk(mu_);
  return hits_;
}

std::vector<std::vector<uint32_t>> find_hint_cuts(const Graph& graph, const NamedInputs& in, const HintChains& chains) {
  const uint32_t N = (uint32_t)graph.nodes.size(), n_hints = graph.tree_depth + 1 + graph.max_out;
  const InputSlots& slots = in.slots;
  std::vector<std::vector<uint32_t>> cuts(n_hints);
  std::vector<uint8_t> match(N, 1);
  std::vector<uint32_t> match_hint(N, 0xFFFFFFFFu);
  bool all = true;
  uint64_t st = 0x9E3779B97F4A7C15ull;
  for (int round = 0; round < 2 && all; round++) {
    std::vector<uint8_t> probe((size_t)graph.inputs_size * 32, 0);
    probe[0] = 1;
    auto put = [&](uint32_t slot) {
      for (int k = 0; k < 31; k++) {
        st = st * 6364136223846793005ull + 1442695040888963407ull;
        probe[32 * (size_t)slot + k] = (uint8_t)(st >> 56);
      }
    };
    put(slots.secret); put(slots.x); put(slots.ext);
    probe[32 * (size_t)slots.limit] = (uint8_t)(100 + round);
    for (uint32_t k = 0; k < in.hint_msgs; k++) probe[32 * (size_t)(in.hint_msg_off + k)] = (uint8_t)(7 + round + 3 * k);
    {
      auto it = graph.input_mapping.find("selectorUsed");
      if (it != graph.input_mapping.end())
        for (uint32_t k = 0; k < it->second.second; k++) probe[32 * (size_t)(it->second.first + k)] = 1;
    }
    for (uint32_t l = 0; l < slots.depth; l++) {
      put(slots.path + l);
      probe[32 * (size_t)(slots.path_idx + l)] = (uint8_t)((l + round) & 1);
    }
    uint32_t perr = 0;
    const std::vector<Fr> val = wl_eval_host(graph, probe.data(), &perr);
    std::vector<Fr> hv(n_hints);
    chains.hints(probe.data(), hv.data());
    all = perr == 0;
    for (uint32_t n = 0; n < N && all; n++) {
      if (!match[n]) continue;
      if (graph.nodes[n].op == G_INPUT || graph.nodes[n].op == G_CONST) { match[n] = 0; continue; }
      uint32_t j = round == 0 ? 0xFFFFFFFFu : match_hint[n];
      if (round == 0) {
        for (uint32_t q = 0; q < n_hints; q++)
          if (val[n] == hv[q]) j = q;
        match_hint[n] = j;
      }
      if (j == 0xFFFFFFFFu || !(val[n] == hv[j])) match[n] = 0;
    }
  }
  for (uint32_t n = 0; n < N && all; n++)
    if (match[n]) cuts[match_hint[n]].push_back(n);
  for (uint32_t j = 0; j < n_hints && all; j++) all = !cuts[j].empty();
  if (!all) cuts.clear();
  return cuts;
}

Wit29Program compile_witness29(const Graph& graph, const std::vector<uint8_t>& is_cut) {
  const uint32_t NONE = 0xFFFFFFFFu;
  const std::vector<GNode>& G = graph.nodes;
  const uint32_t N = (uint32_t)G.size();
  Wit29Program R;
  std::vector<uint32_t>& slot2node = R.slot2node;
  auto is_const = [&](uint32_t o) { return G[o].op == G_CONST; };
  auto nops = [&](const GNode& g) {
    return (g.op == G_INPUT || g.op == G_CONST) ? 0 : (g.op == G_NEG || g.op == G_ID) ? 1 : g.op == G_TERN ? 3 : 2;
  };
  std::vector<uint32_t> uses(N, 0);
  for (uint32_t n = 0; n < N; n++) {
    const uint32_t o[3] = {G[n].a, G[n].b, G[n].c};
    for (int k = 0; k < nops(G[n]); k++) {
      if (o[k] >= n) throw Error("Graph error: node operand refers forward");
      uses[o[k]]++;
    }
  }
  std::vector<uint8_t> is_signal(N, 0);
  for (uint32_t sgn : graph.signals) is_signal[sgn] = 1;
  std::vector<uint32_t> fused_mul(N, NONE);
  std::vector<uint8_t> removed(N, 0);
  for (uint32_t n = 0; n < N; n++) {
    if (G[n].op != G_ADD) continue;
    for (uint32_t m : {G[n].b, G[n].a}) {
      if (G[m].op == G_MUL && uses[m] == 1 && !is_signal[m] && !is_cut[m] && !removed[m] && G[n].a != G[n].b) {
        fused_mul[n] = m;
        removed[m] = 1;
        break;
      }
    }
  }
  struct PNode { uint32_t op, node, src[3]; };
  std::vector<PNode> P;
  std::vector<uint32_t> pidx(N, NONE);
  for (uint32_t n = 0; n < N; n++) {
    if (removed[n]) continue;
    PNode q{G[n].op, n, {G[n].a, G[n].b, G[n].c}};
    if (fused_mul[n] != NONE) {
      const uint32_t m = fused_mul[n];
      q.op = W29_FMA;
      q.src[0] = G[m].a;
      q.src[1] = G[m].b;
      q.src[2] = G[n].a == m ? G[n].b : G[n].a;
    }
    pidx[n] = (uint32_t)P.size();
    P.push_back(q);
  }
  auto pn_ops = [&](const PNode& q) { return q.op == W29_FMA ? 3 : nops(GNode{q.op, 0, 0, 0}); };
  std::vector<uint8_t> store(N, 0);
  for (uint32_t n = 0; n < N; n++) store[n] = is_signal[n] || G[n].op == G_INPUT || is_cut[n];
  for (uint32_t i = 0; i < P.size(); i++)
    for (int k = 0; k < pn_ops(P[i]); k++) {
      const uint32_t o = P[i].src[k];
      if (!is_const(o) && i - pidx[o] >= WIT29_RING) store[o] = 1;
    }
  std::vector<uint32_t> slot_of(N, 0);
  R.store_slot.assign(N, NONE);
  for (uint32_t n = 0; n < N; n++)
    if (store[n] && !removed[n]) {
      slot_of[n] = R.store_slot[n] = (uint32_t)slot2node.size();
      slot2node.push_back(n);
    }
  if (slot2node.size() >= 65536)
    throw Error("graph too large for the witness interpreter: " + std::to_string(slot2node.size()) +
                " stored values, the descriptor holds 16 bits");
  std::vector<GNode29>& prog = R.prog;
  prog.resize(P.size());
  std::vector<double> bnd(N, 1.01);
  for (uint32_t i = 0; i < P.size(); i++) {
    const PNode& q = P[i];
    GNode29 d{};
    uint32_t flags = store[q.node] ? W29_STORE : 0;
    d.a = q.src[0];
    double b = 1.01;
    bool rare = q.op != G_MUL && q.op != G_ADD && q.op != W29_FMA;
    if (q.op != G_INPUT && q.op != G_CONST) {
      auto enc = [&](uint32_t o) -> uint32_t {
        if (is_const(o)) {
          if (G[o].a >= WIT29_LDS_CONSTS) rare = true;
          return OPK_CONST | G[o].a;
        }
        if (i - pidx[o] < WIT29_RING) return OPK_RING | pidx[o];
        rare = true;
        return OPK_FAR | slot_of[o];
      };
      auto bo = [&](uint32_t o) { return is_const(o) ? 1.01 : bnd[o]; };
      const int k = pn_ops(q);
      double bs[3] = {0, 0, 0};
      uint32_t e[3] = {0, 0, 0};
      for (int j = 0; j < k; j++) {
        e[j] = enc(q.src[j]);
        bs[j] = bo(q.src[j]);
      }
      d.a = e[0];
      d.b = e[1];
      d.c = e[2];
      if (q.op == G_MUL) b = 1.0 + 0.006 * bs[0] * bs[1];
      else if (q.op == W29_FMA) b = 1.0 + 0.006 * bs[0] * bs[1] + bs[2];
      else if (q.op == G_ADD) b = bs[0] + bs[1];
      else if (q.op == G_SUB) b = bs[0] + 8.0;
      else if (q.op == G_NEG) b = 8.0;
      else if (q.op == G_TERN) b = std::max(bs[1], bs[2]);
    }
    if (b > WIT29_BMAX) {
      flags |= W29_RED;
      rare = true;
      b = 1.0 + 0.006 * b;
    }
    if (rare) flags |= W29_RARE;
    bnd[q.node] = b;
    d.w0 = q.op | flags | (slot_of[q.node] << 16);
    prog[i] = d;
  }
  R.nprog = (uint32_t)prog.size();
  prog.resize(((size_t)R.nprog / WIT29_CH + 4) * WIT29_CH, GNode29{});
  return R;
}

G1Rows g1_walk_rows(const Zkey& zk, uint32_t NS, uint32_t n, uint32_t ni) {
  const uint32_t SID_R = NS + n, SID_S = SID_R + 1, SID_NRS = SID_R + 2;
  G1Rows R;
  std::vector<G1Affine>& pts = R.pts;
  std::vector<uint32_t>& sids = R.sids;
  std::vector<uint32_t> row_seg;
  auto push = [&](const G1Affine& P, uint32_t sid, uint32_t seg) {
    if (P.is_inf()) return;
    pts.push_back(P);
    sids.push_back(sid);
    row_seg.push_back(seg);
  };
  for (uint32_t i = 0; i < NS; i++) push(zk.a_query[i], i, 0);
  push(zk.alpha_g1, 0, 0);
  push(zk.delta_g1, SID_R, 0);
  for (uint32_t i = 0; i < NS; i++) push(zk.b_g1_query[i], i, 1);
  push(zk.beta_g1, 0, 1);
  push(zk.delta_g1, SID_S, 1);
  for (uint32_t j = 0; j < zk.l_query.size(); j++) push(zk.l_query[j], ni + j, 2);
  for (uint32_t k = 0; k < n; k++) push(zk.h_query[k], NS + k, 2);
  push(zk.delta_g1, SID_NRS, 2);
  {
    std::vector<std::vector<uint32_t>> by_sid(NS);
    for (uint32_t k = 0; k < sids.size(); k++)
      if (sids[k] < NS) by_sid[sids[k]].push_back(k);
    std::vector<uint32_t> order;
    std::vector<uint8_t> taken(sids.size(), 0);
    for (const auto& v : by_sid)
      for (size_t t = 0; t + 1 < v.size(); t += 2) {
        order.push_back(v[t]);
        order.push_back(v[t + 1]);
        taken[v[t]] = taken[v[t + 1]] = 1;
      }
    R.npaired = (uint32_t)order.size();
    for (uint32_t k = 0; k < sids.size(); k++)
      if (!taken[k]) order.push_back(k);
    std::vector<G1Affine> p2(pts.size());
    std::vector<uint32_t> s2(sids.size()), g2(sids.size());
    for (size_t i = 0; i < order.size(); i++) {
      p2[i] = pts[order[i]];
      s2[i] = sids[order[i]];
      g2[i] = row_seg[order[i]];
    }
    pts.swap(p2);
    sids.swap(s2);
    row_seg.swap(g2);
  }
  for (uint32_t k = 0; k < sids.size(); k++)
    R.rows.push_back({k, sids[k], sids[k], row_seg[k], sids[k] >= NS && sids[k] < NS + n});
  std::vector<VRow>& f = R.fused;
  const uint32_t NX = NS + n + 3;
  for (uint32_t k = 0; k < sids.size(); k++) {
    const uint32_t sd = sids[k], sg = row_seg[k];
    const bool is_h = sd >= NS && sd < NS + n;
    if (sg == 0) {
      f.push_back({k, sd, sd, 0, false});
      if (sd < NS) f.push_back({k, sd, NX + sd, 2, false});
    } else if (sg == 1) {
      if (sd < NS) f.push_back({k, sd, NX + NS + sd, 2, false});
    } else if (sd == SID_NRS) {
      f.push_back({k, sd, NX + 2 * NS, 2, false});
    } else {
      f.push_back({k, sd, sd, 2, is_h});
    }
  }
  return R;
}

G2Rows g2_walk_rows(const Zkey& zk, uint32_t NS, uint32_t n) {
  G2Rows R;
  std::vector<uint32_t> sids;
  auto push = [&](const G2Affine& P, uint32_t sid) {
    if (P.is_inf()) return;
    R.pts.push_back(P);
    sids.push_back(sid);
  };
  for (uint32_t i = 0; i < NS; i++) push(zk.b_g2_query[i], i);
  push(zk.beta_g2, 0);
  push(zk.delta_g2, NS + n + 1);
  R.dsid = sids;
  for (uint32_t& v : R.dsid)
    if (v >= NS) v -= n;
  for (uint32_t k = 0; k < sids.size(); k++) R.rows.push_back({k, sids[k], R.dsid[k], 0u, false});
  return R;
}

void make_reduce_ranges(const std::vector<uint32_t>& segfirst, std::vector<ChunkDesc>& groups, std::vector<ChunkDesc>& segs) {
  const uint32_t G = 16;
  for (size_t sgi = 0; sgi + 1 < segfirst.size(); sgi++) {
    uint32_t g0 = (uint32_t)groups.size();
    for (uint32_t c = segfirst[sgi]; c < segfirst[sgi + 1]; c += G)
      groups.push_back({c, std::min(c + G, segfirst[sgi + 1])});
    segs.push_back({g0, (uint32_t)groups.size()});
  }
}

WalkPlan make_walk_plan(const std::vector<VRow>& vrows, uint32_t nseg, uint32_t chunk_pts, int mode,
                        const std::vector<uint8_t>& known, uint32_t npaired, bool pair_chunks, uint32_t block_pts) {
  WalkPlan P;
  const uint32_t NS = (uint32_t)known.size();
  auto roww = [&](uint32_t k, uint32_t h) { return k | (k < npaired ? ROW_PAIRED : 0u) | (h << 31); };
  std::vector<uint32_t> segfirst;
  const bool pairs_here = pair_chunks && npaired > 0;
  auto walked = [&](const VRow& v) {
    const bool is_known = v.sid < NS && known[v.sid];
    return mode == PROVE_FULL || (mode == PROVE_PARTIAL) == is_known;
  };
  struct PairChunk { uint32_t h, sg0, sg1, begin, end; };
  std::vector<PairChunk> pcs;
  if (pairs_here) {
    std::vector<const VRow*> byk(npaired, nullptr);
    for (const VRow& v : vrows)
      if (v.k < npaired) byk[v.k] = &v;
    for (uint32_t h = 0; h < GLV_HALVES; h++)
      for (uint32_t sg0 = 0; sg0 < nseg; sg0++)
        for (uint32_t sg1 = 0; sg1 < nseg; sg1++) {
          const uint32_t first = (uint32_t)P.prows.size();
          for (uint32_t q = 0; q + 1 < npaired; q += 2) {
            const VRow *a = byk[q], *b = byk[q + 1];
            if (!a || !b || a->seg != sg0 || b->seg != sg1) continue;
            if (a->dig_sid != b->dig_sid || a->is_h || b->is_h) throw Error("internal: pair members must share a witness scalar");
            if (!walked(*a)) continue;
            P.prows.push_back(roww(q, h));
            P.prsid.push_back(a->dig_sid);
          }
          for (uint32_t k = first; k < P.prows.size(); k += chunk_pts)
            pcs.push_back({h, sg0, sg1, k, (uint32_t)std::min<size_t>(k + chunk_pts, P.prows.size())});
        }
    P.pout.assign(2 * pcs.size(), 0);
    for (const PairChunk& c : pcs) P.pchunks.push_back({c.begin, c.end});
  }
  for (uint32_t h = 0; h < GLV_HALVES; h++)
    for (uint32_t sg = 0; sg < nseg; sg++) {
      segfirst.push_back((uint32_t)P.chunks.size());
      for (int late = 0; late < 2; late++) {
        uint32_t first = (uint32_t)P.rows.size();
        for (const VRow& v : vrows) {
          if (v.seg != sg || (int)v.is_h != late) continue;
          if (pairs_here && v.k < npaired) continue;
          if (walked(v)) {
            P.rows.push_back(roww(v.k, h));
            P.rsid.push_back(v.dig_sid);
          }
        }
        for (uint32_t k = first; k < P.rows.size(); k += chunk_pts) {
          (late ? P.late_ids : P.early_ids).push_back((uint32_t)P.chunks.size());
          P.chunks.push_back({k, (uint32_t)std::min<size_t>(k + chunk_pts, P.rows.size())});
        }
      }
      for (size_t c = 0; c < pcs.size(); c++)
        for (uint32_t m = 0; m < 2; m++)
          if (pcs[c].h == h && (m ? pcs[c].sg1 : pcs[c].sg0) == sg) {
            P.pout[2 * c + m] = (uint32_t)P.chunks.size();
            P.chunks.push_back({0, 0});
          }
    }
  segfirst.push_back((uint32_t)P.chunks.size());
  make_reduce_ranges(segfirst, P.groups, P.segs);
  P.nseg = nseg * GLV_HALVES;
  for (size_t sgi = 0; sgi + 1 < segfirst.size(); sgi++) {
    P.segchunks.push_back({segfirst[sgi], segfirst[sgi + 1]});
    const uint32_t k = (segfirst[sgi + 1] - segfirst[sgi] + block_pts - 1) / block_pts;
    P.segblocks.push_back({P.nblocks, P.nblocks + k});
    P.nblocks += k;
    P.maxblk = std::max(P.maxblk, k);
  }
  return P;
}

BatchShape batch_shape(const BatchQuery& q, const ProverTuning& T) {
  BatchShape S{};
  const size_t n = q.n;
  const int mode = q.mode;
  S.lone = T.lone >= 0 ? T.lone != 0 : (n <= T.lone_small_max || q.idle);
  S.small = n <= T.lanechunk_max;
  const uint32_t wl_lone_max = q.shared ? std::min(T.witlanes_max, 256u) : T.witlanes_max;
  S.wl_used = q.witlanes_ok && (S.small || (n <= wl_lone_max && S.lone));
  S.cone = mode == PROVE_FINISH && q.handles && q.inputs && S.wl_used && q.cone_ok;
  S.hinted = q.segs_ok && q.inputs && S.wl_used && !S.cone && S.lone && !q.no_hints_now &&
             n <= (q.pre_hints ? HINT_PROOFS : std::max(T.hint_max, T.hint_max_warm));
  S.probe_chains = S.hinted && !q.pre_hints && n > T.hint_max;
  S.early = S.small && mode != PROVE_PARTIAL;
  S.fused = S.lone && n <= 96 && S.early && (mode == PROVE_FULL || (mode == PROVE_FINISH && q.inputs && q.partial_points));
  S.tiny_partial = S.lone && S.small && mode == PROVE_PARTIAL && n <= T.tiny_max && n <= TINY_STRIDE && n <= T.lanechunk_walk_max;
  S.tiny = (S.fused && n <= T.tiny_max && n <= TINY_STRIDE && n <= T.lanechunk_walk_max) || S.tiny_partial;
  S.plan1 = S.tiny ? PLAN_TINY : S.fused ? PLAN_FUSED : S.small ? PLAN_SMALL : PLAN_BIG;
  S.plan2 = S.tiny ? PLAN_TINY : S.small ? PLAN_SMALL : PLAN_BIG;
  S.PB = S.tiny ? TINY_STRIDE : S.small ? q.small_stride : (uint32_t)q.capacity;
  S.walk_lp = S.early && (n > T.lanechunk_walk_max || (!S.lone && n >= 16));
  S.dB = (S.early && !S.walk_lp) ? (uint32_t)n : (uint32_t)q.capacity;
  S.g2_on_front = S.lone && S.early;
  S.values_w = (S.early || S.wl_used) && q.have_values_kernel && q.ni == 6;
  S.ntt_lds = S.small && n <= T.ntt_lg_max && q.logn >= 9 && q.logn <= 18;
  return S;
}

}
```

### zerokit_amd/csrc/prover_plan.h

```cpp
#pragma once
#include <stdint.h>

#include <mutex>
#include <vector>

#include "prover.h"
#include "prover_desc.h"
#include "zkey.h"

namespace rlnamd {

constexpr uint32_t HINT_PROOFS = 64;
constexpr uint32_t TINY_STRIDE = 8;

WinSched make_sched(int c, int wide);

struct NamedInputs {
  InputSlots slots{};
  bool have_values_kernel = false;
  bool have_hint_slots = false;
  uint32_t hint_msg_off = 0, hint_msgs = 1;
};
NamedInputs find_named_inputs(const Graph& graph, uint32_t ni);

class HintChains {
 public:
  struct Probe {
    Fr idc;
    uint64_t fp[2];
    bool found;
  };
  void configure(const NamedInputs& in, uint32_t entries) { in_ = in; entries_ = entries; }
  uint32_t count() const { return in_.slots.depth + 1 + in_.hint_msgs; }
  void probe(const uint8_t* in_le, Probe* pr) const;
  void hints(const uint8_t* in_le, Fr* out, const Probe* pr = nullptr) const;
  uint64_t hits() const;

 private:
  struct Entry {
    uint64_t fp[2] = {0, 0};
    uint64_t stamp = 0;
    std::vector<Fr> chain;
  };
  NamedInputs in_;
  uint32_t entries_ = 0;
  mutable std::mutex mu_;
  mutable std::vector<Entry> cache_;
  mutable uint64_t clock_ = 0, hits_ = 0;
};

std::vector<std::vector<uint32_t>> find_hint_cuts(const Graph& graph, const NamedInputs& in, const HintChains& chains);

struct Wit29Program {
  std::vector<GNode29> prog;
  uint32_t nprog = 0;
  std::vector<uint32_t> slot2node;
  std::vector<uint32_t> store_slot;
};
Wit29Program compile_witness29(const Graph& graph, const std::vector<uint8_t>& is_cut);

struct VRow {
  uint32_t k, sid, dig_sid, seg;
  bool is_h;
};
struct G1Rows {
  std::vector<G1Affine> pts;
  std::vector<uint32_t> sids;
  uint32_t npaired = 0;
  std::vector<VRow> rows, fused;
};
struct G2Rows {
  std::vector<G2Affine> pts;
  std::vector<uint32_t> dsid;
  std::vector<VRow> rows;
};
G1Rows g1_walk_rows(const Zkey& zk, uint32_t NS, uint32_t n, uint32_t ni);
G2Rows g2_walk_rows(const Zkey& zk, uint32_t NS, uint32_t n);

void make_reduce_ranges(const std::vector<uint32_t>& segfirst, std::vector<ChunkDesc>& groups, std::vector<ChunkDesc>& segs);

struct WalkPlan {
  std::vector<uint32_t> rows, rsid;
  std::vector<ChunkDesc> chunks, groups, segs, segchunks;
  std::vector<uint32_t> early_ids, late_ids;
  uint32_t nseg = 0;
  std::vector<uint32_t> prows, prsid, pout;
  std::vector<ChunkDesc> pchunks;
  std::vector<ChunkDesc> segblocks;
  uint32_t nblocks = 0, maxblk = 0;
};
constexpr uint32_t GLV_HALVES = 2;
WalkPlan make_walk_plan(const std::vector<VRow>& vrows, uint32_t nseg, uint32_t chunk_pts, int mode,
                        const std::vector<uint8_t>& known, uint32_t npaired = 0, bool pair_chunks = false,
                        uint32_t block_pts = SUM_TREE_LANES);

enum WalkPlanKind { PLAN_BIG = 0, PLAN_SMALL, PLAN_FUSED, PLAN_TINY };
struct BatchQuery {
  size_t n = 0;
  int mode = PROVE_FULL;
  bool inputs = false, partial_points = false, handles = false, pre_hints = false;
  bool idle = true;
  bool shared = false;
  bool no_hints_now = false;
  bool witlanes_ok = false, segs_ok = false, cone_ok = false, have_values_kernel = false;
  uint32_t ni = 0;
  int logn = 0;
  size_t capacity = 0;
  uint32_t small_stride = 64;
};
struct BatchShape {
  bool lone, small, wl_used, cone, hinted, early, fused, tiny_partial, tiny, walk_lp, g2_on_front, values_w, ntt_lds;
  bool probe_chains;
  WalkPlanKind plan1, plan2;
  uint32_t PB, dB;
};
BatchShape batch_shape(const BatchQuery& q, const ProverTuning& T);

}
```

Measured before the change: 20150.

## Replace ad-hoc prover streams with stage-to-stream plan over four streams

Collapses the eight hand-managed HIP streams into four indexed streams and adds a table-driven plan that assigns each proving stage to a stream per batch shape and inserts event waits only on edges that cross streams. The aim is fewer redundant cross-stream waits and less launch/sync overhead, with the stage placement chosen per shape. In exchange the previous alternating-stream trick for back-to-back batches is gone, so overlap between consecutive batches may drop, and any dependency left out of the plan would be a correctness risk.

```diff
diff --git a/zerokit_amd/csrc/prover.hip b/zerokit_amd/csrc/prover.hip
--- a/zerokit_amd/csrc/prover.hip
+++ b/zerokit_amd/csrc/prover.hip
@@ -66,6 +66,7 @@
   hipEvent_t free_event() const { return wiped ? evZ : evC; }
   size_t n = 0;
   uint32_t dB = 0, PB = 0, nch1 = 0, nch2 = 0;
+  uint8_t wipe_st = STREAM_F;
 };
 
 static std::atomic<int> g_provers_on_device[64];
@@ -147,10 +148,7 @@
 };
 
 struct Prover::Impl {
-  hipStream_t sA = nullptr, sAb = nullptr, sA2 = nullptr, sB = nullptr, sB2 = nullptr, sC = nullptr;
-  hipStream_t sV = nullptr;
-  hipStream_t sW = nullptr;
-  uint32_t seq = 0;
+  hipStream_t st[PROVER_STREAMS] = {};
   float ms[PROVER_STAGES] = {0};
   DevBuf<unsigned long long> walk_clk;
   ProverTuning tune;
@@ -255,6 +253,7 @@
     const size_t n = S.n ? S.n : batch_cap;
     const size_t B = batch_cap;
     if (!n) return;
+    const hipStream_t sW = st[S.wipe_st];
     RLN_HIP(hipStreamWaitEvent(sW, S.evC, 0));
     WipeRanges WR{};
     auto flush = [&]() {
@@ -315,14 +314,7 @@
   }
 
   void sync_all() {
-    RLN_HIP(hipStreamSynchronize(sA));
-    RLN_HIP(hipStreamSynchronize(sAb));
-    RLN_HIP(hipStreamSynchronize(sV));
-    RLN_HIP(hipStreamSynchronize(sA2));
-    RLN_HIP(hipStreamSynchronize(sB));
-    if (sB2) RLN_HIP(hipStreamSynchronize(sB2));
-    RLN_HIP(hipStreamSynchronize(sC));
-    RLN_HIP(hipStreamSynchronize(sW));
+    for (hipStream_t s : st) RLN_HIP(hipStreamSynchronize(s));
   }
 };
 
@@ -465,19 +457,15 @@
   {
     int lo = 0, hi = 0;
     RLN_HIP(hipDeviceGetStreamPriorityRange(&lo, &hi));
-    RLN_HIP(hipStreamCreateWithPriority(&D.sW, hipStreamNonBlocking, hi));
-    RLN_HIP(hipStreamCreateWithPriority(&D.sA, hipStreamNonBlocking, hi));
-    RLN_HIP(hipStreamCreateWithPriority(&D.sA2, hipStreamNonBlocking, hi));
-    RLN_HIP(hipStreamCreateWithPriority(&D.sAb, hipStreamNonBlocking, hi));
-    RLN_HIP(hipStreamCreateWithPriority(&D.sV, hipStreamNonBlocking, hi));
-    RLN_HIP(hipStreamCreateWithPriority(&D.sB, hipStreamNonBlocking, lo));
-    RLN_HIP(hipStreamCreateWithPriority(&D.sC, hipStreamNonBlocking, hi));
+    RLN_HIP(hipStreamCreateWithPriority(&D.st[STREAM_C], hipStreamNonBlocking, hi));
+    RLN_HIP(hipStreamCreateWithPriority(&D.st[STREAM_F], hipStreamNonBlocking, hi));
+    RLN_HIP(hipStreamCreateWithPriority(&D.st[STREAM_Q], hipStreamNonBlocking, hi));
+    RLN_HIP(hipStreamCreateWithPriority(&D.st[STREAM_W], hipStreamNonBlocking, lo));
     D.nslot = std::min(std::max(D.tune.slots, 2), (int)Impl::NSLOT);
     D.walk_clk.alloc(4);
     RLN_HIP(hipMemset(D.walk_clk.p, 0, 4 * sizeof(unsigned long long)));
-    RLN_HIP(hipStreamCreateWithPriority(&D.sB2, hipStreamNonBlocking, lo));
-  }
-  hipStream_t s = D.sB;
+  }
+  hipStream_t s = D.st[STREAM_W];
 
   RLN_HIP(hipFuncSetAttribute((const void*)(k_sum_tree<Fq2, G2Acc29>), hipFuncAttributeMaxDynamicSharedMemorySize, SUM_TREE_LDS_G2));
   RLN_HIP(hipFuncSetAttribute((const void*)(k_sum_blocks<Fq2, G2Acc29>), hipFuncAttributeMaxDynamicSharedMemorySize, SUM_TREE_LDS_G2));
@@ -732,16 +720,16 @@
 Prover::~Prover() {
   if (!d_) return;
   Impl& D = *d_;
-  for (hipStream_t st : {D.sA, D.sAb, D.sA2, D.sB, D.sB2, D.sC, D.sV, D.sW})
+  for (hipStream_t st : D.st)
     if (st) (void)hipStreamSynchronize(st);
   try {
-    if (D.sW) {
+    if (D.st[STREAM_C]) {
       for (int k = 0; k < D.nslot; k++)
         if (D.slot[k].used && !D.slot[k].wiped && D.slot[k].evC) D.wipe_slot(D.slot[k], D.slot[k].ticket == 0);
       if (D.cone_cache.p)
-        hipLaunchKernelGGL(k_wipe_bytes, dim3(div_up(D.cone_cache.bytes() / 16, 256)), dim3(64), 0, D.sW, D.cone_cache.p,
+        hipLaunchKernelGGL(k_wipe_bytes, dim3(div_up(D.cone_cache.bytes() / 16, 256)), dim3(64), 0, D.st[STREAM_C], D.cone_cache.p,
                            (uint32_t)(D.cone_cache.bytes() / 16));
-      (void)hipStreamSynchronize(D.sW);
+      for (hipStream_t st : D.st) (void)hipStreamSynchronize(st);
     }
   } catch (...) {
   }
@@ -762,7 +750,7 @@
   }
   for (hipEvent_t e : {D.evConeSaved, D.evConeRead, D.evConeRead2})
     if (e) (void)hipEventDestroy(e);
-  for (hipStream_t st : {D.sA, D.sAb, D.sA2, D.sB, D.sB2, D.sC, D.sV, D.sW})
+  for (hipStream_t st : D.st)
     if (st) (void)hipStreamDestroy(st);
 }
 
@@ -774,9 +762,9 @@
   if (n > B_) throw Error("batch larger than the prover workspace (max_batch)");
   Impl& D = *d_;
   D.sync_all();
-  RLN_HIP(hipMemcpyAsync(D.inputs.p, inputs, n * D.NI * 32, hipMemcpyHostToDevice, D.sA));
-  RLN_HIP(hipMemcpyAsync(D.rs.p, rs, n * 64, hipMemcpyHostToDevice, D.sA));
-  RLN_HIP(hipStreamSynchronize(D.sA));
+  RLN_HIP(hipMemcpyAsync(D.inputs.p, inputs, n * D.NI * 32, hipMemcpyHostToDevice, D.st[STREAM_F]));
+  RLN_HIP(hipMemcpyAsync(D.rs.p, rs, n * 64, hipMemcpyHostToDevice, D.st[STREAM_F]));
+  RLN_HIP(hipStreamSynchronize(D.st[STREAM_F]));
 }
 
 void Prover::upload_witness(size_t n, const uint8_t* w_le) {
@@ -785,8 +773,8 @@
   D.sync_all();
   size_t words = n * (size_t)D.NS * 8;
   if (D.wgiven.n < words) D.wgiven.alloc(words);
-  RLN_HIP(hipMemcpyAsync(D.wgiven.p, w_le, words * 4, hipMemcpyHostToDevice, D.sA));
-  RLN_HIP(hipStreamSynchronize(D.sA));
+  RLN_HIP(hipMemcpyAsync(D.wgiven.p, w_le, words * 4, hipMemcpyHostToDevice, D.st[STREAM_F]));
+  RLN_HIP(hipStreamSynchronize(D.st[STREAM_F]));
   D.wgiven_n = n;
 }
 
@@ -868,12 +856,14 @@
     cached++;
   }
   if (cached) {
-    RLN_HIP(hipStreamWaitEvent(D.sW, S.evC, 0));
-    hipLaunchKernelGGL(k_cone_save, dim3(div_up(D.cone_nk * 3, 256), (uint32_t)cached), dim3(256), 0, D.sW, S.V29.p, D.cone_rows.p,
+    const hipStream_t sW = D.st[S.wipe_st];
+    RLN_HIP(hipStreamWaitEvent(sW, S.evC, 0));
+    RLN_HIP(hipStreamWaitEvent(sW, D.evConeSaved, 0));
+    hipLaunchKernelGGL(k_cone_save, dim3(div_up(D.cone_nk * 3, 256), (uint32_t)cached), dim3(256), 0, sW, S.V29.p, D.cone_rows.p,
                        D.cone_nk, (uint32_t)B_, S.h_cone, D.cone_cache.p, D.cone_stride);
-    launch_pp_powers(D.sW, S.pp_out.p, S.h_cone, D.cone_cache.p, D.cone_stride, D.cone_nk * 3, (uint32_t)cached);
+    launch_pp_powers(sW, S.pp_out.p, S.h_cone, D.cone_cache.p, D.cone_stride, D.cone_nk * 3, (uint32_t)cached);
     RLN_HIP(hipGetLastError());
-    RLN_HIP(hipEventRecord(D.evConeSaved, D.sW));
+    RLN_HIP(hipEventRecord(D.evConeSaved, sW));
   }
   collect(ticket, n, nullptr, nullptr, errors, nullptr, partial320, true);
 }
@@ -882,23 +872,25 @@
   Impl& D = *d_;
   if (!D.cone_cap || !handles) return;
   bool any = false;
+  const hipStream_t sW = D.st[STREAM_C];
   for (size_t i = 0; i < n; i++) {
     const uint32_t e = D.cone_entry(handles[i]);
     if (e == 0xFFFFFFFFu) continue;
     if (!any) {
-      RLN_HIP(hipStreamWaitEvent(D.sW, D.evConeRead, 0));
-      RLN_HIP(hipStreamWaitEvent(D.sW, D.evConeRead2, 0));
+      RLN_HIP(hipStreamWaitEvent(sW, D.evConeRead, 0));
+      RLN_HIP(hipStreamWaitEvent(sW, D.evConeRead2, 0));
+      RLN_HIP(hipStreamWaitEvent(sW, D.evConeSaved, 0));
     }
     any = true;
     uint4* at = D.cone_cache.p + (size_t)e * D.cone_stride;
-    hipLaunchKernelGGL(k_wipe_bytes, dim3(div_up(D.cone_stride, 256)), dim3(64), 0, D.sW, at, D.cone_stride);
+    hipLaunchKernelGGL(k_wipe_bytes, dim3(div_up(D.cone_stride, 256)), dim3(64), 0, sW, at, D.cone_stride);
     D.cone_live[e] = 0;
     D.cone_gen[e]++;
     D.cone_free.push_back(e);
   }
   if (any) {
     RLN_HIP(hipGetLastError());
-    RLN_HIP(hipEventRecord(D.evConeSaved, D.sW));
+    RLN_HIP(hipEventRecord(D.evConeSaved, sW));
   }
 }
 
@@ -925,17 +917,16 @@
   out[7] = D.witlanes.ok ? D.witlanes.nsteps : 0;
   if (!D.cone_cap) return;
   sync();
-  RLN_HIP(hipStreamSynchronize(D.sW));
   DevBuf<unsigned long long> cnt(1);
-  RLN_HIP(hipMemsetAsync(cnt.p, 0, cnt.bytes(), D.sC));
+  RLN_HIP(hipMemsetAsync(cnt.p, 0, cnt.bytes(), D.st[STREAM_C]));
   for (uint32_t e = 0; e < D.cone_cap; e++)
     if (!D.cone_live[e])
-      hipLaunchKernelGGL(k_count_nonzero16, dim3(64), dim3(256), 0, D.sC, (const uint4*)(D.cone_cache.p + (size_t)e * D.cone_stride),
+      hipLaunchKernelGGL(k_count_nonzero16, dim3(64), dim3(256), 0, D.st[STREAM_C], (const uint4*)(D.cone_cache.p + (size_t)e * D.cone_stride),
                          (size_t)D.cone_stride, cnt.p);
   RLN_HIP(hipGetLastError());
   unsigned long long h = 0;
-  RLN_HIP(hipMemcpyAsync(&h, cnt.p, sizeof h, hipMemcpyDeviceToHost, D.sC));
-  RLN_HIP(hipStreamSynchronize(D.sC));
+  RLN_HIP(hipMemcpyAsync(&h, cnt.p, sizeof h, hipMemcpyDeviceToHost, D.st[STREAM_C]));
+  RLN_HIP(hipStreamSynchronize(D.st[STREAM_C]));
   out[3] = h;
 }
 
@@ -1002,7 +993,7 @@
   if (ticket == 0) {
     D.sync_all();
     if (D.last) D.wipe_slot(*D.last, true);
-    RLN_HIP(hipStreamSynchronize(D.sW));
+    D.sync_all();
     return;
   }
   for (int k = 0; k < D.nslot; k++)
@@ -1173,12 +1164,15 @@
   S.mode = mode;
   S.ticket = streamed ? ++D.tickets : 0;
   D.cur = (D.cur + 1) % D.nslot;
-  const uint32_t sq = D.seq++;
-  const bool idle = !D.last || hipEventQuery(D.last->evC) == hipSuccess;
-  (void)hipGetLastError();
-  hipStream_t sA = (!idle && (sq & 1)) ? D.sAb : D.sA;
+  const StreamPlan SP = stream_plan(sh, mode, streamed);
+  S.wipe_st = SP.stream[STAGE_WIPE];
+  auto on = [&](StageId stage) { return D.st[SP.stream[stage]]; };
+  auto after = [&](StageId to, StageId from, hipEvent_t ev) {
+    if (SP.stream[to] != SP.stream[from]) RLN_HIP(hipStreamWaitEvent(on(to), ev, 0));
+  };
+  const hipStream_t sA = on(STAGE_INTERP), sA2 = on(STAGE_QUOT), sB = on(STAGE_G1_EARLY), sL = on(STAGE_G1_LATE),
+                    sC = on(STAGE_SUM_C), sP = on(STAGE_PP), sS = on(STAGE_SUM_A);
   const uint32_t B = (uint32_t)B_, nb = (uint32_t)n;
-  hipStream_t sA2 = !early ? D.sA2 : sh.g2_on_front ? D.sB2 : sA;
   const uint32_t pg = div_up(nb, 64);
   const uint32_t nbp = pg * 64;
   auto d2h = [&](void* host, const void* dev, size_t bytes, hipStream_t st) {
@@ -1205,17 +1199,24 @@
                          nullptr, ids);
     }
   };
-  if (S.used) RLN_HIP(hipStreamWaitEvent(sA, S.free_event(), 0));
+  if (S.used) {
+    bool waits[PROVER_STREAMS] = {};
+    for (uint8_t stage : SP.free_waits) {
+      if (!waits[SP.stream[stage]]) RLN_HIP(hipStreamWaitEvent(D.st[SP.stream[stage]], S.free_event(), 0));
+      waits[SP.stream[stage]] = true;
+    }
+  }
   if (streamed) {
     auto h2d = [&](void* dst, const uint8_t* src, size_t bytes) {
-      hipLaunchKernelGGL(k_stage_in, dim3(div_up(bytes / 16, 64)), dim3(64), 0, sA, (const uint4*)src, (uint4*)dst,
+      hipLaunchKernelGGL(k_stage_in, dim3(div_up(bytes / 16, 64)), dim3(64), 0, on(STAGE_STAGING), (const uint4*)src, (uint4*)dst,
                          (uint32_t)(bytes / 16));
     };
     h2d(S.inputs.p, S.h_in, n * (size_t)D.NI * 32);
     h2d(S.rs.p, S.h_in + B_ * (size_t)D.NI * 32, n * 64);
     if (h_pp320) h2d(S.pp_in.p, S.h_in + B_ * ((size_t)D.NI * 32 + 64), n * 320);
     RLN_HIP(hipGetLastError());
-    RLN_HIP(hipEventRecord(S.evU, sA));
+    RLN_HIP(hipEventRecord(S.evU, on(STAGE_STAGING)));
+    after(STAGE_INTERP, STAGE_STAGING, S.evU);
   }
   const bool marks = !small;
   S.marked = marks;
@@ -1238,18 +1239,17 @@
     D.hinted_batches++;
   }
   if (fused && mode == PROVE_FINISH) {
-    if (S.used) RLN_HIP(hipStreamWaitEvent(D.sC, S.free_event(), 0));
-    RLN_HIP(hipStreamWaitEvent(D.sC, S.evU, 0));
+    after(STAGE_PP, STAGE_STAGING, S.evU);
     if (cone) {
-      RLN_HIP(hipStreamWaitEvent(D.sC, D.evConeSaved, 0));
-      launch_pp_smul(D.sC, D.cone_cache.p, S.h_cone, D.cone_stride, D.cone_nk * 3, rs_p, S.prod.p, nb);
-      RLN_HIP(hipEventRecord(D.evConeRead2, D.sC));
+      RLN_HIP(hipStreamWaitEvent(sP, D.evConeSaved, 0));
+      launch_pp_smul(sP, D.cone_cache.p, S.h_cone, D.cone_stride, D.cone_nk * 3, rs_p, S.prod.p, nb);
+      RLN_HIP(hipEventRecord(D.evConeRead2, sP));
     } else {
-      launch_pp_powers(D.sC, pp_p, D.iota96.p, S.pp_pow.p, PP_POWERS16, 0, nb);
-      launch_pp_smul(D.sC, S.pp_pow.p, D.iota96.p, PP_POWERS16, 0, rs_p, S.prod.p, nb);
+      launch_pp_powers(sP, pp_p, D.iota96.p, S.pp_pow.p, PP_POWERS16, 0, nb);
+      launch_pp_smul(sP, S.pp_pow.p, D.iota96.p, PP_POWERS16, 0, rs_p, S.prod.p, nb);
     }
     RLN_HIP(hipGetLastError());
-    RLN_HIP(hipEventRecord(S.evP, D.sC));
+    RLN_HIP(hipEventRecord(S.evP, sP));
   }
   MARK(1, sA);
   if (cone) {
@@ -1285,27 +1285,27 @@
   }
   RLN_HIP(hipEventRecord(S.evX, sA));
   if (early) {
-    hipStream_t sR1 = sA, sR3 = lone ? D.sB : sA;
+    hipStream_t sR1 = sA, sR3 = lone ? sB : sA;
     hipLaunchKernelGGL(k_recode, dim3(div_up(D.NS + 3, 64), nb), dim3(64, 1), 0, sR1, S.V.p, D.sig2node.p, D.NS,
                        S.abc.p, D.n, rs_p, D.ws, D.ws2, S.digits.p, S.digits2.p, B, nb, 1u, 1u, dB);
     if (lone) {
       RLN_HIP(hipEventRecord(S.evW, sA));
-      RLN_HIP(hipStreamWaitEvent(D.sB, S.evW, 0));
+      after(STAGE_G1_EARLY, STAGE_INTERP, S.evW);
     }
     if (fused)
       hipLaunchKernelGGL(k_recode, dim3(div_up(2 * D.NS + 1, 64), nb), dim3(64, 1), 0, sR3, S.V.p, D.sig2node.p, D.NS,
                          S.abc.p, D.n, rs_p, D.ws, D.ws2, S.digits.p, S.digits2.p, B, nb, 3u, 1u, dB);
     if (!lone) {
       RLN_HIP(hipEventRecord(S.evW, sA));
-      RLN_HIP(hipStreamWaitEvent(D.sB, S.evW, 0));
-      RLN_HIP(hipStreamWaitEvent(D.sB2, S.evW, 0));
-    }
-    MARK(14, D.sB);
-    walk1(D.sB, P1.early_ids.p, P1.n_early);
-    RLN_HIP(hipEventRecord(S.evE, D.sB));
+      after(STAGE_G1_EARLY, STAGE_INTERP, S.evW);
+      after(STAGE_G2, STAGE_INTERP, S.evW);
+    }
+    MARK(14, sB);
+    walk1(sB, P1.early_ids.p, P1.n_early);
+    RLN_HIP(hipEventRecord(S.evE, sB));
   }
   MARK(2, sA);
-  if (sA2 != sA) RLN_HIP(hipStreamWaitEvent(sA2, S.evX, 0));
+  after(STAGE_QUOT, STAGE_INTERP, S.evX);
   MARK(12, sA2);
   if (mode != PROVE_PARTIAL) {
     CsrView A{D.a_ptr.p, D.a_col.p, D.a_coef.p}, Bm{D.b_ptr.p, D.b_col.p, D.b_coef.p};
@@ -1343,22 +1343,17 @@
   MARK(6, sR);
   if (!early) {
     RLN_HIP(hipEventRecord(S.evA, sA2));
-    RLN_HIP(hipStreamWaitEvent(D.sB, S.evA, 0));
-    MARK(14, D.sB);
-  }
-  hipStream_t s2 = sh.g2_on_front ? sA : D.sB2;
-  if (!early) {
-    RLN_HIP(hipEventRecord(S.evR, D.sB));
-    RLN_HIP(hipStreamWaitEvent(D.sB2, S.evR, 0));
-  }
+    after(STAGE_G1_LATE, STAGE_QUOT, S.evA);
+    MARK(14, sL);
+  }
+  hipStream_t s2 = on(STAGE_G2);
   if (early) {
-    walk1(sA2, P1.late_ids.p, P1.n_late);
-    RLN_HIP(hipEventRecord(S.evR, sA2));
-    RLN_HIP(hipStreamWaitEvent(D.sB, S.evR, 0));
+    walk1(sL, P1.late_ids.p, P1.n_late);
+    RLN_HIP(hipEventRecord(S.evR, sL));
   } else {
-    walk1(D.sB, nullptr, P1.nchunks);
-  }
-  MARK(7, D.sB);
+    walk1(sL, nullptr, P1.nchunks);
+  }
+  MARK(7, sL);
   MARK(11, s2);
   if (P2.nchunks) {
     uint32_t blocks = div_up(P2.nchunks, 8) * 8 * pg;
@@ -1379,17 +1374,13 @@
                          D.walk_clk.p ? D.walk_clk.p + 2 : nullptr);
   }
   MARK(8, s2);
-  RLN_HIP(hipEventRecord(S.evB, D.sB));
+  if (!early) RLN_HIP(hipEventRecord(S.evB, on(STAGE_G1_DONE)));
   RLN_HIP(hipEventRecord(S.evB2, s2));
-  hipStream_t sV = D.sV;
-  if (S.used) {
-    RLN_HIP(hipStreamWaitEvent(D.sC, S.free_event(), 0));
-    RLN_HIP(hipStreamWaitEvent(sV, S.free_event(), 0));
-  }
-  if (streamed) RLN_HIP(hipStreamWaitEvent(sV, S.evU, 0));
+  hipStream_t sV = on(STAGE_VALUES);
+  if (streamed) after(STAGE_VALUES, STAGE_STAGING, S.evU);
   MARK(0, sV);
   if (sh.values_w) {
-    RLN_HIP(hipStreamWaitEvent(sV, S.evX, 0));
+    after(STAGE_VALUES, STAGE_INTERP, S.evX);
     hipLaunchKernelGGL(k_values_from_witness, dim3(pg, 5), dim3(64), 0, sV, S.V.p, D.sig2node.p, B, nbp, S.values.p);
   } else if (D.have_values_kernel)
     hipLaunchKernelGGL(k_proof_values, dim3(pg), dim3(64), 0, sV, in_p, D.NI, D.slots, poseidon_view(2),
@@ -1397,7 +1388,7 @@
   MARK(13, sV);
   const bool fin_pp = mode == PROVE_FINISH;
   const TaskSel all4 = task_sel({0, 1, 2, 3}), all3 = task_sel({0, 1, 2});
-  hipStream_t sF = D.sC;
+  const hipStream_t sF = on(STAGE_COPY);
   auto sum1 = [&](hipStream_t st, std::initializer_list<uint32_t> segs) {
     const TaskSel sel = task_sel(segs);
     const uint32_t ns = (uint32_t)segs.size();
@@ -1420,91 +1411,87 @@
     }
   };
   if (early) {
-    RLN_HIP(hipStreamWaitEvent(D.sA2, S.evE, 0));
+    after(STAGE_SUM_A, STAGE_G1_EARLY, S.evE);
     if (fused) {
-      sum1(D.sA2, {0, 3});
-      if (fin_pp) hipLaunchKernelGGL(k_add_partial, dim3(pg, 1), dim3(64), 0, D.sA2, S.sums1.p, S.sums2.p, pp_p, B, nbp, task_sel({0}), (const G1XYZZ*)nullptr);
+      sum1(sS, {0, 3});
+      if (fin_pp) hipLaunchKernelGGL(k_add_partial, dim3(pg, 1), dim3(64), 0, sS, S.sums1.p, S.sums2.p, pp_p, B, nbp, task_sel({0}), (const G1XYZZ*)nullptr);
     } else {
-      sum1(D.sA2, {0, 1, 3, 4});
-      if (fin_pp) hipLaunchKernelGGL(k_add_partial, dim3(pg, 2), dim3(64), 0, D.sA2, S.sums1.p, S.sums2.p, pp_p, B, nbp, task_sel({0, 1}), (const G1XYZZ*)nullptr);
-      hipLaunchKernelGGL(k_glv_fold, dim3(pg, 2), dim3(64), 0, D.sA2, S.sums1.p, S.sums2.p, 3u, B, nbp, task_sel({0, 1}));
-      hipLaunchKernelGGL(k_fin_affine, dim3(pg, 2), dim3(64), 0, D.sA2, S.sums1.p, S.sums2.p, S.affA.p, S.affB1.p,
+      sum1(sS, {0, 1, 3, 4});
+      if (fin_pp) hipLaunchKernelGGL(k_add_partial, dim3(pg, 2), dim3(64), 0, sS, S.sums1.p, S.sums2.p, pp_p, B, nbp, task_sel({0, 1}), (const G1XYZZ*)nullptr);
+      hipLaunchKernelGGL(k_glv_fold, dim3(pg, 2), dim3(64), 0, sS, S.sums1.p, S.sums2.p, 3u, B, nbp, task_sel({0, 1}));
+      hipLaunchKernelGGL(k_fin_affine, dim3(pg, 2), dim3(64), 0, sS, S.sums1.p, S.sums2.p, S.affA.p, S.affB1.p,
                          S.affB2.p, B, nbp, task_sel({0, 1}));
-      launch_fin_smul29(D.sA2, S.affA.p, S.affB1.p, rs_p, S.prod.p, B, nb);
+      launch_fin_smul29(sS, S.affA.p, S.affB1.p, rs_p, S.prod.p, B, nb);
     }
     RLN_HIP(hipGetLastError());
-    RLN_HIP(hipEventRecord(S.evA, D.sA2));
-    hipStream_t sG = lone ? s2 : D.sC;
-    if (!lone) RLN_HIP(hipStreamWaitEvent(D.sC, S.evB2, 0));
+    RLN_HIP(hipEventRecord(S.evA, sS));
+    const hipStream_t sG = on(STAGE_SUM_G2);
+    after(STAGE_SUM_G2, STAGE_G2, S.evB2);
     sum2(sG);
     if (fin_pp) hipLaunchKernelGGL(k_add_partial, dim3(pg, 1), dim3(64), 0, sG, S.sums1.p, S.sums2.p, pp_p, B, nbp, task_sel({3}), (const G1XYZZ*)nullptr);
     hipLaunchKernelGGL(k_fin_out_b2, dim3(pg), dim3(64), 0, sG, S.sums2.p, S.coords.p, S.comp.p, B, nbp);
-    if (lone) RLN_HIP(hipEventRecord(S.evB2, s2));
+    if (lone) RLN_HIP(hipEventRecord(S.evB2, sG));
     RLN_HIP(hipEventRecord(S.evV, sV));
-    hipStream_t sAC = lone ? sA2 : sF;
-    if (lone) {
-      sF = sA;
-      MARK(9, sF);
-      RLN_HIP(hipStreamWaitEvent(sAC, S.evE, 0));
-    } else {
-      MARK(9, sF);
-      RLN_HIP(hipStreamWaitEvent(sF, S.evB, 0));
-    }
+    const hipStream_t sAC = sC;
+    MARK(9, sF);
+    after(STAGE_SUM_C, STAGE_G1_EARLY, S.evE);
+    after(STAGE_SUM_C, STAGE_G1_LATE, S.evR);
     sum1(sAC, {2, 5});
     if (fin_pp) hipLaunchKernelGGL(k_add_partial, dim3(pg, 1), dim3(64), 0, sAC, S.sums1.p, S.sums2.p, pp_p, B, nbp, task_sel({2}), (const G1XYZZ*)nullptr);
     if (fin_pp && fused) {
-      RLN_HIP(hipStreamWaitEvent(sAC, S.evP, 0));
+      after(STAGE_SUM_C, STAGE_PP, S.evP);
       hipLaunchKernelGGL(k_add_partial, dim3(pg, 1), dim3(64), 0, sAC, S.sums1.p, S.sums2.p, pp_p, B, nbp, task_sel({4}), (const G1XYZZ*)S.prod.p);
     }
-    RLN_HIP(hipStreamWaitEvent(sAC, S.evA, 0));
+    after(STAGE_SUM_C, STAGE_SUM_A, S.evA);
     if (fused)
       hipLaunchKernelGGL(k_fin_out_ac_fused, dim3(pg), dim3(64), 0, sAC, S.sums1.p, S.affA.p, S.coords.p, S.comp.p, B, nbp);
     else
       hipLaunchKernelGGL(k_fin_out_ac, dim3(pg), dim3(64), 0, sAC, S.sums1.p, S.prod.p, S.affA.p, S.coords.p, S.comp.p, B, nbp);
     if (lone) {
       RLN_HIP(hipEventRecord(S.evA, sAC));
-      RLN_HIP(hipStreamWaitEvent(sF, S.evA, 0));
-    }
-    RLN_HIP(hipStreamWaitEvent(sF, S.evV, 0));
+      after(STAGE_COPY, STAGE_SUM_C, S.evA);
+    }
+    after(STAGE_COPY, STAGE_VALUES, S.evV);
   } else {
     if (tiny_partial) {
-      sum2(s2);
-      RLN_HIP(hipEventRecord(S.evB2, s2));
+      after(STAGE_SUM_G2, STAGE_G2, S.evB2);
+      sum2(on(STAGE_SUM_G2));
+      RLN_HIP(hipEventRecord(S.evB2, on(STAGE_SUM_G2)));
     }
     RLN_HIP(hipEventRecord(S.evV, sV));
-    RLN_HIP(hipStreamWaitEvent(D.sC, S.evV, 0));
-    RLN_HIP(hipStreamWaitEvent(D.sC, S.evB, 0));
-    if (tiny_partial) sum1(D.sC, {0, 1, 2, 3, 4, 5});
-    RLN_HIP(hipStreamWaitEvent(D.sC, S.evB2, 0));
-    MARK(9, D.sC);
+    after(STAGE_SUM_C, STAGE_VALUES, S.evV);
+    after(STAGE_SUM_C, STAGE_G1_DONE, S.evB);
+    if (tiny_partial) sum1(sC, {0, 1, 2, 3, 4, 5});
+    after(STAGE_SUM_C, tiny_partial ? STAGE_SUM_G2 : STAGE_G2, S.evB2);
+    MARK(9, sC);
   }
   if (early || tiny_partial) {
   } else if (small) {
-    sum1(D.sC, {0, 1, 2, 3, 4, 5});
-    sum2(D.sC);
+    sum1(sC, {0, 1, 2, 3, 4, 5});
+    sum2(sC);
   } else {
     if (P1.ngroups)
-      hipLaunchKernelGGL(k_sum_ranges<Fq>, dim3(pg, P1.ngroups), dim3(64), 0, D.sC, S.part1.p, P1.groups.p, P1.ngroups,
+      hipLaunchKernelGGL(k_sum_ranges<Fq>, dim3(pg, P1.ngroups), dim3(64), 0, sC, S.part1.p, P1.groups.p, P1.ngroups,
                          S.grp1.p, B, nbp);
     if (P2.ngroups)
-      hipLaunchKernelGGL(k_sum_ranges<Fq2>, dim3(pg, P2.ngroups), dim3(64), 0, D.sC, S.part2.p, P2.groups.p, P2.ngroups,
+      hipLaunchKernelGGL(k_sum_ranges<Fq2>, dim3(pg, P2.ngroups), dim3(64), 0, sC, S.part2.p, P2.groups.p, P2.ngroups,
                          S.grp2.p, B, nbp);
-    hipLaunchKernelGGL(k_sum_ranges<Fq>, dim3(pg, P1.nseg), dim3(64), 0, D.sC, S.grp1.p, P1.segs.p, P1.nseg, S.sums1.p, B, nbp);
-    hipLaunchKernelGGL(k_sum_ranges<Fq2>, dim3(pg, P2.nseg), dim3(64), 0, D.sC, S.grp2.p, P2.segs.p, P2.nseg, S.sums2.p, B, nbp);
+    hipLaunchKernelGGL(k_sum_ranges<Fq>, dim3(pg, P1.nseg), dim3(64), 0, sC, S.grp1.p, P1.segs.p, P1.nseg, S.sums1.p, B, nbp);
+    hipLaunchKernelGGL(k_sum_ranges<Fq2>, dim3(pg, P2.nseg), dim3(64), 0, sC, S.grp2.p, P2.segs.p, P2.nseg, S.sums2.p, B, nbp);
   }
   if (!early)
-    hipLaunchKernelGGL(k_glv_fold, dim3(pg, 4), dim3(64), 0, D.sC, S.sums1.p, S.sums2.p, 3u, B, nbp, all4);
+    hipLaunchKernelGGL(k_glv_fold, dim3(pg, 4), dim3(64), 0, sC, S.sums1.p, S.sums2.p, 3u, B, nbp, all4);
   if (mode == PROVE_PARTIAL) {
-    hipLaunchKernelGGL(k_partial_out, dim3(pg, 4), dim3(64), 0, D.sC, S.sums1.p, S.sums2.p, S.pp_out.p, B, nbp);
+    hipLaunchKernelGGL(k_partial_out, dim3(pg, 4), dim3(64), 0, sC, S.sums1.p, S.sums2.p, S.pp_out.p, B, nbp);
     RLN_HIP(hipGetLastError());
-    d2h(S.h_pp, S.pp_out.p, n * 320, D.sC);
+    d2h(S.h_pp, S.pp_out.p, n * 320, sC);
   } else {
     if (!early) {
       if (mode == PROVE_FINISH)
-        hipLaunchKernelGGL(k_add_partial, dim3(pg, 4), dim3(64), 0, D.sC, S.sums1.p, S.sums2.p, pp_p, B, nbp, all4, (const G1XYZZ*)nullptr);
-      hipLaunchKernelGGL(k_fin_affine, dim3(pg, 3), dim3(64), 0, D.sC, S.sums1.p, S.sums2.p, S.affA.p, S.affB1.p,
+        hipLaunchKernelGGL(k_add_partial, dim3(pg, 4), dim3(64), 0, sC, S.sums1.p, S.sums2.p, pp_p, B, nbp, all4, (const G1XYZZ*)nullptr);
+      hipLaunchKernelGGL(k_fin_affine, dim3(pg, 3), dim3(64), 0, sC, S.sums1.p, S.sums2.p, S.affA.p, S.affB1.p,
                          S.affB2.p, B, nbp, all3);
-      hipLaunchKernelGGL(k_fin_smul, dim3(pg, 2), dim3(64), 0, D.sC, S.affA.p, S.affB1.p, rs_p, S.tbl.p, S.prod.p, B,
+      hipLaunchKernelGGL(k_fin_smul, dim3(pg, 2), dim3(64), 0, sC, S.affA.p, S.affB1.p, rs_p, S.tbl.p, S.prod.p, B,
                          nbp);
       hipLaunchKernelGGL(k_fin_out, dim3(pg), dim3(64), 0, sF, S.sums1.p, S.prod.p, S.affA.p, S.affB2.p, S.coords.p,
                          S.comp.p, B, nbp);
@@ -1556,8 +1543,8 @@
   if (n > B_) throw Error("batch larger than the prover workspace (max_batch)");
   Impl& D = *d_;
   D.sync_all();
-  RLN_HIP(hipMemcpyAsync(D.pp_in.p, coords320, n * 320, hipMemcpyHostToDevice, D.sA));
-  RLN_HIP(hipStreamSynchronize(D.sA));
+  RLN_HIP(hipMemcpyAsync(D.pp_in.p, coords320, n * 320, hipMemcpyHostToDevice, D.st[STREAM_F]));
+  RLN_HIP(hipStreamSynchronize(D.st[STREAM_F]));
 }
 
 void Prover::download_partial(size_t n, uint8_t* coords320) {
@@ -1591,8 +1578,8 @@
   if (!D.last) throw Error("no resident run to read from");
   Slot& S = *D.last;
   std::vector<uint32_t> coords(n * 64);
-  RLN_HIP(hipMemcpyAsync(coords.data(), S.coords.p, n * 256, hipMemcpyDeviceToHost, D.sC));
-  RLN_HIP(hipStreamSynchronize(D.sC));
+  RLN_HIP(hipMemcpyAsync(coords.data(), S.coords.p, n * 256, hipMemcpyDeviceToHost, D.st[STREAM_C]));
+  RLN_HIP(hipStreamSynchronize(D.st[STREAM_C]));
   std::vector<uint8_t> pub;
   const bool from_public = !D.have_values_kernel && D.ni == 6;
   if (from_public) fetch_public(n, &pub);
@@ -1621,11 +1608,11 @@
   Slot& S = *(Slot*)slot;
   const uint32_t npub = D.ni - 1;
   DevBuf<uint32_t> tmp(n * npub * 8);
-  hipLaunchKernelGGL(k_public_signals, dim3(div_up(n, 64), div_up(npub, 4)), dim3(64, 4), 0, D.sC, S.V.p,
+  hipLaunchKernelGGL(k_public_signals, dim3(div_up(n, 64), div_up(npub, 4)), dim3(64, 4), 0, D.st[STREAM_C], S.V.p,
                      D.sig2node.p, npub, (uint32_t)B_, (uint32_t)n, tmp.p);
   out_le->resize(n * npub * 32);
-  RLN_HIP(hipMemcpyAsync(out_le->data(), tmp.p, out_le->size(), hipMemcpyDeviceToHost, D.sC));
-  RLN_HIP(hipStreamSynchronize(D.sC));
+  RLN_HIP(hipMemcpyAsync(out_le->data(), tmp.p, out_le->size(), hipMemcpyDeviceToHost, D.st[STREAM_C]));
+  RLN_HIP(hipStreamSynchronize(D.st[STREAM_C]));
 }
 
 void Prover::fetch_witness(size_t p, std::vector<uint8_t>* w_le) {
@@ -1633,11 +1620,11 @@
   sync();
   if (!D.last || p >= B_) throw Error("no resident run to read from");
   DevBuf<uint32_t> tmp((size_t)D.NS * 8);
-  hipLaunchKernelGGL(k_gather_col, dim3(div_up(D.NS, 256)), dim3(256), 0, D.sC, D.last->V.p, D.sig2node.p, D.NS,
+  hipLaunchKernelGGL(k_gather_col, dim3(div_up(D.NS, 256)), dim3(256), 0, D.st[STREAM_C], D.last->V.p, D.sig2node.p, D.NS,
                      (uint32_t)B_, (uint32_t)p, tmp.p);
   w_le->resize((size_t)D.NS * 32);
-  RLN_HIP(hipMemcpyAsync(w_le->data(), tmp.p, w_le->size(), hipMemcpyDeviceToHost, D.sC));
-  RLN_HIP(hipStreamSynchronize(D.sC));
+  RLN_HIP(hipMemcpyAsync(w_le->data(), tmp.p, w_le->size(), hipMemcpyDeviceToHost, D.st[STREAM_C]));
+  RLN_HIP(hipStreamSynchronize(D.st[STREAM_C]));
 }
 
 void Prover::fetch_h(size_t p, std::vector<uint8_t>* h_le) {
@@ -1645,11 +1632,11 @@
   sync();
   if (!D.last || p >= B_) throw Error("no resident run to read from");
   DevBuf<uint32_t> tmp((size_t)D.n * 8);
-  hipLaunchKernelGGL(k_gather_col, dim3(div_up(D.n, 256)), dim3(256), 0, D.sC, D.last->abc.p, (const uint32_t*)nullptr,
+  hipLaunchKernelGGL(k_gather_col, dim3(div_up(D.n, 256)), dim3(256), 0, D.st[STREAM_C], D.last->abc.p, (const uint32_t*)nullptr,
                      D.n, (uint32_t)B_, (uint32_t)p, tmp.p);
   h_le->resize((size_t)D.n * 32);
-  RLN_HIP(hipMemcpyAsync(h_le->data(), tmp.p, h_le->size(), hipMemcpyDeviceToHost, D.sC));
-  RLN_HIP(hipStreamSynchronize(D.sC));
+  RLN_HIP(hipMemcpyAsync(h_le->data(), tmp.p, h_le->size(), hipMemcpyDeviceToHost, D.st[STREAM_C]));
+  RLN_HIP(hipStreamSynchronize(D.st[STREAM_C]));
 }
 
 void Prover::residue(uint64_t out[RESIDUE_FIELDS]) {
@@ -1658,10 +1645,10 @@
   if (!D.last) throw Error("no run to read from");
   Slot& S = *D.last;
   DevBuf<unsigned long long> cnt(RESIDUE_FIELDS);
-  RLN_HIP(hipMemsetAsync(cnt.p, 0, cnt.bytes(), D.sC));
+  RLN_HIP(hipMemsetAsync(cnt.p, 0, cnt.bytes(), D.st[STREAM_C]));
   auto count = [&](int k, const void* p, size_t bytes) {
     if (p && bytes >= 16)
-      hipLaunchKernelGGL(k_count_nonzero16, dim3(2048), dim3(256), 0, D.sC, (const uint4*)p, bytes / 16, cnt.p + k);
+      hipLaunchKernelGGL(k_count_nonzero16, dim3(2048), dim3(256), 0, D.st[STREAM_C], (const uint4*)p, bytes / 16, cnt.p + k);
   };
   count(0, S.digits.p, S.digits.bytes());
   count(1, S.digits2.p, S.digits2.bytes());
@@ -1677,8 +1664,8 @@
   count(5, S.rs.p, S.rs.bytes());
   RLN_HIP(hipGetLastError());
   unsigned long long h[RESIDUE_FIELDS];
-  RLN_HIP(hipMemcpyAsync(h, cnt.p, sizeof h, hipMemcpyDeviceToHost, D.sC));
-  RLN_HIP(hipStreamSynchronize(D.sC));
+  RLN_HIP(hipMemcpyAsync(h, cnt.p, sizeof h, hipMemcpyDeviceToHost, D.st[STREAM_C]));
+  RLN_HIP(hipStreamSynchronize(D.st[STREAM_C]));
   for (int k = 0; k < RESIDUE_FIELDS; k++) out[k] = h[k];
 }
 
diff --git a/zerokit_amd/csrc/prover_plan.cpp b/zerokit_amd/csrc/prover_plan.cpp
--- a/zerokit_amd/csrc/prover_plan.cpp
+++ b/zerokit_amd/csrc/prover_plan.cpp
@@ -524,4 +524,116 @@
   return S;
 }
 
-}
+StreamPlan stream_plan(const BatchShape& sh, int mode, bool streamed) {
+  StreamPlan P{};
+  const bool early = sh.early, lone_early = sh.early && sh.g2_on_front;
+  for (int s = 0; s < PROVER_STAGE_COUNT; s++) P.runs[s] = true;
+  P.runs[STAGE_STAGING] = streamed;
+  P.runs[STAGE_PP] = sh.fused && mode == PROVE_FINISH;
+  P.runs[STAGE_G1_EARLY] = P.runs[STAGE_SUM_A] = early;
+  P.runs[STAGE_G1_DONE] = !early;
+  P.runs[STAGE_SUM_G2] = early || sh.tiny_partial;
+  uint8_t* st = P.stream;
+  st[STAGE_STAGING] = st[STAGE_INTERP] = STREAM_F;
+  st[STAGE_PP] = STREAM_C;
+  st[STAGE_G1_EARLY] = st[STAGE_G1_DONE] = STREAM_W;
+  st[STAGE_SUM_A] = STREAM_C;
+  if (!sh.small) {
+    st[STAGE_VALUES] = STREAM_F;
+    st[STAGE_QUOT] = STREAM_Q;
+    st[STAGE_G1_LATE] = st[STAGE_G2] = st[STAGE_SUM_G2] = STREAM_W;
+    st[STAGE_SUM_C] = st[STAGE_COPY] = STREAM_C;
+    st[STAGE_WIPE] = STREAM_F;
+  } else if (!early) {
+    st[STAGE_VALUES] = STREAM_C;
+    st[STAGE_QUOT] = st[STAGE_G2] = st[STAGE_SUM_G2] = STREAM_Q;
+    st[STAGE_G1_LATE] = STREAM_W;
+    st[STAGE_SUM_C] = st[STAGE_COPY] = STREAM_C;
+    st[STAGE_WIPE] = sh.lone ? STREAM_C : STREAM_F;
+  } else if (lone_early) {
+    st[STAGE_VALUES] = STREAM_C;
+    st[STAGE_QUOT] = st[STAGE_G1_LATE] = st[STAGE_SUM_C] = STREAM_Q;
+    st[STAGE_G2] = st[STAGE_SUM_G2] = st[STAGE_COPY] = STREAM_F;
+    st[STAGE_WIPE] = STREAM_C;
+  } else {
+    st[STAGE_VALUES] = STREAM_C;
+    st[STAGE_QUOT] = st[STAGE_G1_LATE] = STREAM_F;
+    st[STAGE_G2] = STREAM_Q;
+    st[STAGE_SUM_G2] = st[STAGE_SUM_C] = st[STAGE_COPY] = STREAM_C;
+    st[STAGE_WIPE] = STREAM_F;
+  }
+  auto edge = [&](int from, int to) {
+    if (P.runs[from] && P.runs[to]) P.edges.push_back({(uint8_t)from, (uint8_t)to});
+  };
+  edge(STAGE_STAGING, STAGE_INTERP);
+  edge(STAGE_STAGING, STAGE_PP);
+  edge(STAGE_STAGING, STAGE_VALUES);
+  edge(STAGE_INTERP, STAGE_QUOT);
+  if (sh.values_w) edge(STAGE_INTERP, STAGE_VALUES);
+  if (early) {
+    edge(STAGE_INTERP, STAGE_G1_EARLY);
+    edge(STAGE_INTERP, STAGE_G2);
+    edge(STAGE_G1_EARLY, STAGE_SUM_A);
+    edge(STAGE_G2, STAGE_SUM_G2);
+    edge(STAGE_G1_EARLY, STAGE_SUM_C);
+    edge(STAGE_G1_LATE, STAGE_SUM_C);
+    edge(STAGE_PP, STAGE_SUM_C);
+    edge(STAGE_SUM_A, STAGE_SUM_C);
+    if (lone_early) edge(STAGE_SUM_C, STAGE_COPY);
+    edge(STAGE_VALUES, STAGE_COPY);
+  } else {
+    edge(STAGE_QUOT, STAGE_G1_LATE);
+    edge(STAGE_QUOT, STAGE_G2);
+    edge(STAGE_G2, STAGE_SUM_G2);
+    edge(STAGE_VALUES, STAGE_SUM_C);
+    edge(STAGE_G1_DONE, STAGE_SUM_C);
+    edge(sh.tiny_partial ? STAGE_SUM_G2 : STAGE_G2, STAGE_SUM_C);
+  }
+  P.free_waits = {(uint8_t)(streamed ? STAGE_STAGING : STAGE_INTERP), STAGE_VALUES, STAGE_SUM_C};
+  if (P.runs[STAGE_PP]) P.free_waits.push_back(STAGE_PP);
+  return P;
+}
+
+std::vector<StageDep> stage_deps(const BatchShape& sh, int mode, bool streamed) {
+  std::vector<StageDep> d;
+  const bool early = sh.early;
+  auto dep = [&](int w, int r, const char* what) { d.push_back({(uint8_t)w, (uint8_t)r, what}); };
+  if (streamed) {
+    dep(STAGE_STAGING, STAGE_INTERP, "inputs");
+    if (!sh.values_w) dep(STAGE_STAGING, STAGE_VALUES, "inputs");
+    dep(STAGE_STAGING, STAGE_QUOT, "r, s");
+    if (sh.fused && mode == PROVE_FINISH) dep(STAGE_STAGING, STAGE_PP, "r, s, partial points");
+  }
+  if (mode != PROVE_PARTIAL) dep(STAGE_INTERP, STAGE_QUOT, "witness");
+  if (sh.values_w) dep(STAGE_INTERP, STAGE_VALUES, "witness");
+  dep(STAGE_INTERP, STAGE_COPY, "error flags");
+  dep(STAGE_VALUES, STAGE_COPY, "values");
+  if (early) {
+    dep(STAGE_INTERP, STAGE_G1_EARLY, "witness digits (G1)");
+    dep(STAGE_INTERP, STAGE_G2, "witness digits (G2)");
+    dep(STAGE_QUOT, STAGE_G1_LATE, "h digits");
+    dep(STAGE_G1_EARLY, STAGE_SUM_A, "part1 (A, B1)");
+    dep(STAGE_G1_EARLY, STAGE_SUM_C, "part1 (C, early rows)");
+    dep(STAGE_G1_LATE, STAGE_SUM_C, "part1 (C, h rows)");
+    dep(STAGE_G2, STAGE_SUM_G2, "part2");
+    dep(STAGE_SUM_A, STAGE_SUM_C, "A affine, s A, r B1");
+    if (sh.fused && mode == PROVE_FINISH) dep(STAGE_PP, STAGE_SUM_C, "s pi_a + r rho");
+    dep(STAGE_SUM_G2, STAGE_COPY, "B's bytes");
+    dep(STAGE_SUM_C, STAGE_COPY, "A's and C's bytes");
+  } else {
+    dep(STAGE_INTERP, STAGE_QUOT, "witness (recode)");
+    dep(STAGE_QUOT, STAGE_G1_LATE, "digits (G1)");
+    dep(STAGE_QUOT, STAGE_G2, "digits (G2)");
+    dep(STAGE_G1_LATE, STAGE_SUM_C, "part1");
+    if (sh.tiny_partial) {
+      dep(STAGE_G2, STAGE_SUM_G2, "part2");
+      dep(STAGE_SUM_G2, STAGE_SUM_C, "sums2");
+    } else {
+      dep(STAGE_G2, STAGE_SUM_C, "part2");
+    }
+    dep(STAGE_SUM_C, STAGE_COPY, "proof bytes / partial points");
+  }
+  return d;
+}
+
+}
diff --git a/zerokit_amd/csrc/prover_plan.h b/zerokit_amd/csrc/prover_plan.h
--- a/zerokit_amd/csrc/prover_plan.h
+++ b/zerokit_amd/csrc/prover_plan.h
@@ -116,4 +116,43 @@
 };
 BatchShape batch_shape(const BatchQuery& q, const ProverTuning& T);
 
+enum StreamId { STREAM_F = 0, STREAM_Q, STREAM_W, STREAM_C, PROVER_STREAMS };
+enum StageId {
+  STAGE_STAGING = 0,
+  STAGE_PP,
+  STAGE_INTERP,
+  STAGE_G1_EARLY,
+  STAGE_QUOT,
+  STAGE_G1_LATE,
+  STAGE_G1_DONE,
+  STAGE_G2,
+  STAGE_VALUES,
+  STAGE_SUM_A,
+  STAGE_SUM_G2,
+  STAGE_SUM_C,
+  STAGE_COPY,
+  STAGE_WIPE,
+  PROVER_STAGE_COUNT
+};
+struct StageEdge {
+  uint8_t from, to;
+};
+struct StreamPlan {
+  uint8_t stream[PROVER_STAGE_COUNT];
+  bool runs[PROVER_STAGE_COUNT];
+  std::vector<StageEdge> edges;
+  std::vector<uint8_t> free_waits;
+  bool has_edge(int from, int to) const {
+    for (const StageEdge& e : edges)
+      if (e.from == from && e.to == to) return true;
+    return false;
+  }
+};
+StreamPlan stream_plan(const BatchShape& sh, int mode, bool streamed);
+struct StageDep {
+  uint8_t writer, reader;
+  const char* what;
+};
+std::vector<StageDep> stage_deps(const BatchShape& sh, int mode, bool streamed);
+
 }
```

Result: faster. 22770 (median of 6 runs) (+13.0%).
